# CarperAI/trlx

Measured on AMD Instinct MI355X. Metric: ppo_samples_per_sec, higher is better.
Workload: dtype bf16

## Files before the change

### trlx_amd/csrc/attn_host.h

```cpp
#pragma once

#include <ATen/ATen.h>

#include <string>
#include <type_traits>
#include <utility>

#include "dispatch.h"


template <int... Ds>
struct HeadDims {};
constexpr HeadDims<64, 96, 128, 256> kFlashHeadDims{};
constexpr HeadDims<64, 128> kSeq2SeqFlashHeadDims{};
constexpr HeadDims<32, 64, 96, 128, 256> kDecodeHeadDims{};
constexpr HeadDims<64, 128> kSeq2SeqDecodeHeadDims{};


template <int... Ds, typename F>
void dispatch_head_dim(HeadDims<Ds...>, int D, const char* op, F&& f) {
  const bool found = (... || (D == Ds ? (f(std::integral_constant<int, Ds>{}), true) : false));
  if (found) return;
  const int dims[] = {Ds...};
  const int n = sizeof...(Ds);
  std::string list;
  for (int i = 0; i < n; ++i)
    list += (i == 0 ? "" : i + 1 == n ? " or " : ", ") + std::to_string(dims[i]);
  TORCH_CHECK(false, op, ": head dim must be ", list, ", got ", D);
}

template <typename F>
void dispatch_flash_mode(int D, bool alibi, bool s2s_any, bool causal, bool rel_bias,
                         bool key_mask, const char* op, F&& f) {
  constexpr std::true_type yes{};
  constexpr std::false_type no{};
  if (s2s_any) {
    dispatch_head_dim(kSeq2SeqFlashHeadDims, D, op, [&](auto d) {
      dispatch_bool(causal, [&](auto ca) {
        dispatch_bool(rel_bias, [&](auto rb) {
          dispatch_bool(key_mask, [&](auto km) {
            constexpr bool plain =
                decltype(ca)::value && !decltype(rb)::value && !decltype(km)::value;
            if constexpr (!plain) f(d, no, ca, rb, km);
            else TORCH_INTERNAL_ASSERT(false, op, ": seq2seq dispatch without a seq2seq mode");
          });
        });
      });
    });
    return;
  }
  dispatch_head_dim(kFlashHeadDims, D, op, [&](auto d) {
    dispatch_bool(alibi, [&](auto al) { f(d, al, yes, no, no); });
  });
}


inline std::pair<at::Tensor, const int*> optional_int_ptr(const c10::optional<at::Tensor>& opt,
                                                          const at::Tensor& like, long B,
                                                          const char* op, const char* what) {
  if (!opt.has_value()) return {at::Tensor(), nullptr};
  TORCH_CHECK(opt->device() == like.device(), op, ": ", what,
              " must live on the same device as the inputs");
  TORCH_CHECK(opt->dtype() == at::kInt && opt->numel() == B, op, ": ", what,
              " must be int32 with one element per batch row (", B, "), got ", opt->dtype(),
              " x ", opt->numel());
  at::Tensor t = opt->contiguous();
  return {t, t.data_ptr<int>()};
}

inline const float* alibi_slopes_ptr(const c10::optional<at::Tensor>& slopes,
                                     const at::Tensor& like, long num_q_heads,
                                     const char* op) {
  if (!slopes.has_value()) return nullptr;
  TORCH_CHECK(slopes->dtype() == at::kFloat && slopes->is_contiguous(), op,
              ": alibi_slopes must be contiguous fp32");
  TORCH_CHECK(slopes->device() == like.device(), op,
              ": alibi_slopes must live on the same device as the inputs");
  TORCH_CHECK(slopes->numel() == num_q_heads, op, ": alibi_slopes needs one slope per query head (",
              num_q_heads, "), got ", slopes->numel());
  return slopes->data_ptr<float>();
}

struct Seq2SeqArgs {
  const float* rel_bias = nullptr;
  int bias_len = 0;
  int bias_zero = 0;
  const unsigned char* key_mask = nullptr;
  bool any = false;
};

inline Seq2SeqArgs seq2seq_args(const c10::optional<at::Tensor>& rel_bias, long bias_zero,
                                const c10::optional<at::Tensor>& key_mask, bool causal,
                                bool has_key_starts, bool has_alibi, const at::Tensor& like,
                                long B, long num_q_heads, long Tq, long Tk, long start_pos,
                                long D, const char* op) {
  Seq2SeqArgs a;
  if (rel_bias.has_value()) {
    TORCH_CHECK(!has_alibi, op, ": rel_bias and alibi_slopes are mutually exclusive");
    TORCH_CHECK(rel_bias->dtype() == at::kFloat && rel_bias->is_contiguous() &&
                    rel_bias->dim() == 2 && rel_bias->size(0) == num_q_heads,
                op, ": rel_bias must be contiguous fp32 [Hq, L]");
    TORCH_CHECK(rel_bias->device() == like.device(), op,
                ": rel_bias must live on the same device as the inputs");
    const long L = rel_bias->size(1);
    TORCH_CHECK(bias_zero - (start_pos + Tq - 1) >= 0 && bias_zero + Tk - 1 < L, op,
                ": rel_bias [Hq, ", L, "] with bias_zero ", bias_zero,
                " does not cover queries ", start_pos, "..", start_pos + Tq - 1, " x keys 0..",
                Tk - 1);
    a.rel_bias = rel_bias->data_ptr<float>();
    a.bias_len = (int)L;
    a.bias_zero = (int)bias_zero;
  }
  if (key_mask.has_value()) {
    TORCH_CHECK(!has_key_starts, op, ": key_mask and key_starts are mutually exclusive");
    TORCH_CHECK(key_mask->dtype() == at::kByte && key_mask->is_contiguous() &&
                    key_mask->dim() == 2 && key_mask->size(0) == B && key_mask->size(1) == Tk,
                op, ": key_mask must be contiguous uint8 [B, Tk]");
    TORCH_CHECK(key_mask->device() == like.device(), op,
                ": key_mask must live on the same device as the inputs");
    TORCH_CHECK(Tk > 0, op, ": key_mask needs at least one key");
    a.key_mask = key_mask->data_ptr<unsigned char>();
  }
  a.any = a.rel_bias != nullptr || a.key_mask != nullptr || !causal;
  if (a.any) {
    TORCH_CHECK(!has_alibi, op, ": key_mask / non-causal attention do not combine with alibi_slopes");
    TORCH_CHECK(D == 64 || D == 128, op,
                ": rel_bias / key_mask / non-causal attention need head dim 64 or 128, got ", D);
  }
  return a;
}
```

### trlx_amd/csrc/bindings.cpp

```cpp
#include <torch/extension.h>

std::vector<at::Tensor> logprobs_fwd(const at::Tensor& logits, const at::Tensor& labels);
at::Tensor logprobs_bwd(const at::Tensor& logits, const at::Tensor& labels, const at::Tensor& lse,
                        const at::Tensor& gout);
std::vector<at::Tensor> rmsnorm_fwd(const at::Tensor& x, const at::Tensor& w, double eps,
                                    const c10::optional<at::Tensor>& res);
std::vector<at::Tensor> rmsnorm_bwd(const at::Tensor& x, const at::Tensor& w,
                                    const at::Tensor& invr, const at::Tensor& dy,
                                    const c10::optional<at::Tensor>& dres);
std::vector<at::Tensor> layernorm_fwd(const at::Tensor& x, const at::Tensor& w,
                                      const c10::optional<at::Tensor>& b, double eps,
                                      const c10::optional<at::Tensor>& res);
std::vector<at::Tensor> layernorm_bwd(const at::Tensor& x, const at::Tensor& w,
                                      const at::Tensor& mean, const at::Tensor& invstd,
                                      const at::Tensor& dy,
                                      const c10::optional<at::Tensor>& dres);
at::Tensor rope_fwd(const at::Tensor& x, const at::Tensor& cos, const at::Tensor& sin,
                    const at::Tensor& pos, bool interleaved, bool inverse, long rot);
std::vector<at::Tensor> gae(const at::Tensor& values, const at::Tensor& rewards, double gamma,
                            double lam);
at::Tensor sum_count(const at::Tensor& x);
at::Tensor normalize(const at::Tensor& x, const at::Tensor& mean, const at::Tensor& var,
                     bool shift_mean);
std::vector<at::Tensor> ppo_loss(const at::Tensor& logprobs, const at::Tensor& values,
                                 const at::Tensor& old_logprobs, const at::Tensor& old_values,
                                 const at::Tensor& advantages, const at::Tensor& returns,
                                 const at::Tensor& mask, double cliprange, double cliprange_value,
                                 double vf_coef);
at::Tensor gumbel_sample(const at::Tensor& logits, double temperature,
                         const c10::optional<at::Tensor>& thresholds, long seed, long offset);
at::Tensor gumbel_sample_dev(const at::Tensor& logits, double temperature,
                             const c10::optional<at::Tensor>& thresholds, long seed,
                             const at::Tensor& offset);
at::Tensor decode_prep(const at::Tensor& qkv, at::Tensor& kcache, at::Tensor& vcache,
                       const c10::optional<at::Tensor>& cos, const c10::optional<at::Tensor>& sin,
                       const c10::optional<at::Tensor>& key_starts, const at::Tensor& cache_idx,
                       long num_heads, long rot, bool interleaved);
std::vector<at::Tensor> qkv_prep_fwd(const at::Tensor& qkv, long num_heads, long num_kv_heads,
                                     long head_dim, const c10::optional<at::Tensor>& cos,
                                     const c10::optional<at::Tensor>& sin,
                                     const c10::optional<at::Tensor>& pos, double qscale,
                                     long rot, bool interleaved);
at::Tensor qkv_prep_bwd(const at::Tensor& dq, const at::Tensor& dk, const at::Tensor& dv,
                        const c10::optional<at::Tensor>& cos, const c10::optional<at::Tensor>& sin,
                        const c10::optional<at::Tensor>& pos, double qscale, long rot,
                        bool interleaved);
at::Tensor causal_softmax_fwd(const at::Tensor& scores, long start_pos,
                              const c10::optional<at::Tensor>& key_starts);
at::Tensor causal_softmax_bwd(const at::Tensor& probs, const at::Tensor& dprobs);
at::Tensor attention_decode(const at::Tensor& q, const at::Tensor& kc, const at::Tensor& vc,
                            const at::Tensor& seq_lens, double scale,
                            const c10::optional<at::Tensor>& seq_starts,
                            const c10::optional<at::Tensor>& alibi_slopes);
at::Tensor lm_logprobs_v2(const at::Tensor& hidden, const at::Tensor& weight,
                          const at::Tensor& labels);
at::Tensor skinny_gemm(const at::Tensor& a, const at::Tensor& w,
                       const c10::optional<at::Tensor>& bias, long act);
at::Tensor skinny_gemm_fp8(const at::Tensor& a, const at::Tensor& w8, const at::Tensor& wscale,
                           const c10::optional<at::Tensor>& bias, long act);
std::vector<at::Tensor> lm_logprobs_v2_with_lse(const at::Tensor& hidden,
                                                const at::Tensor& weight,
                                                const at::Tensor& labels, bool want_lse);
at::Tensor ce_dlogits(const at::Tensor& hidden, const at::Tensor& weight,
                      const at::Tensor& labels, const at::Tensor& lse, const at::Tensor& dlp);
std::vector<at::Tensor> linear_gather_lse_fwd(const at::Tensor& x, const at::Tensor& w,
                                              const at::Tensor& bias, const at::Tensor& idx);
at::Tensor linear_gather_lse_bwd(const at::Tensor& x, const at::Tensor& w,
                                 const at::Tensor& bias, const at::Tensor& idx,
                                 const at::Tensor& lse, const at::Tensor& g_val,
                                 const at::Tensor& g_lse);
at::Tensor fused_decode_attention(const at::Tensor& qkv, at::Tensor& kcache, at::Tensor& vcache,
                                  const at::Tensor& seq_lens,
                                  const c10::optional<at::Tensor>& seq_starts,
                                  const c10::optional<at::Tensor>& cos,
                                  const c10::optional<at::Tensor>& sin,
                                  const at::Tensor& cache_idx, long rot, bool interleaved,
                                  double scale,
                                  const c10::optional<at::Tensor>& alibi_slopes);
void decode_advance(const at::Tensor& tok, at::Tensor& out_tokens, at::Tensor& cur_tok,
                    at::Tensor& finished, at::Tensor& rng_offset, at::Tensor& step_col,
                    at::Tensor& cache_idx, at::Tensor& seq_lens, at::Tensor& pos_ids,
                    const c10::optional<at::Tensor>& key_starts, long eos, long pad);
at::Tensor lm_logprobs(const at::Tensor& hidden, const at::Tensor& weight,
                       const at::Tensor& labels);
void fused_adamw(at::Tensor& p, at::Tensor& master, const at::Tensor& g, at::Tensor& m,
                 at::Tensor& v, long step, double lr, double beta1, double beta2, double eps,
                 double weight_decay, double grad_scale);
void stage_gemm(const at::Tensor& a, const at::Tensor& w, const c10::optional<at::Tensor>& bias,
                at::Tensor& c, const c10::optional<at::Tensor>& nstats,
                const c10::optional<at::Tensor>& nw, const c10::optional<at::Tensor>& nb,
                bool norm_rms, double eps, long act, const c10::optional<at::Tensor>& resid,
                const c10::optional<at::Tensor>& out_stats);
void embed_stats(const at::Tensor& wte, const c10::optional<at::Tensor>& wpe,
                 const at::Tensor& cur_tok, const at::Tensor& pos_ids, long pos_offset,
                 at::Tensor& x, at::Tensor& stats, at::Tensor& packed);
void lm_sample(const at::Tensor& x, const at::Tensor& wlm, const c10::optional<at::Tensor>& blm,
               const at::Tensor& nstats, const at::Tensor& nw,
               const c10::optional<at::Tensor>& nb, at::Tensor& packed, bool norm_rms,
               double eps, double temperature, long seed, const at::Tensor& rng_offset);
void advance_packed(const at::Tensor& packed, at::Tensor& out_tokens, at::Tensor& cur_tok,
                    at::Tensor& finished, at::Tensor& rng_offset, at::Tensor& step_col,
                    at::Tensor& cache_idx, at::Tensor& seq_lens, at::Tensor& pos_ids,
                    const c10::optional<at::Tensor>& key_starts, long eos, long pad);
void stage_gemm_v2(const at::Tensor& a, const at::Tensor& w, const c10::optional<at::Tensor>& bias,
                   at::Tensor& c, bool norm, const c10::optional<at::Tensor>& nw,
                   const c10::optional<at::Tensor>& nb, bool norm_rms, double eps, long act,
                   const c10::optional<at::Tensor>& resid,
                   const c10::optional<at::Tensor>& pstats_out);
void stage_gemm_v3(const at::Tensor& a, const at::Tensor& w, const c10::optional<at::Tensor>& bias,
                   at::Tensor& c, const c10::optional<at::Tensor>& pstats, long nparts,
                   const c10::optional<at::Tensor>& nw, const c10::optional<at::Tensor>& nb,
                   bool norm_rms, double eps, long act,
                   const c10::optional<at::Tensor>& pstats_out);
at::Tensor flash_prefill(const at::Tensor& q, const at::Tensor& k, const at::Tensor& v,
                         const c10::optional<at::Tensor>& key_starts, long start_pos,
                         double scale, long tk,
                         const c10::optional<at::Tensor>& alibi_slopes,
                         const c10::optional<at::Tensor>& rel_bias, long bias_zero,
                         const c10::optional<at::Tensor>& key_mask, bool causal);
std::vector<at::Tensor> flash_prefill_lse(const at::Tensor& q, const at::Tensor& k,
                                          const at::Tensor& v,
                                          const c10::optional<at::Tensor>& key_starts,
                                          long start_pos, double scale, long tk,
                                          bool want_lse,
                                          const c10::optional<at::Tensor>& alibi_slopes,
                                          const c10::optional<at::Tensor>& rel_bias, long bias_zero,
                                          const c10::optional<at::Tensor>& key_mask, bool causal);
std::vector<at::Tensor> flash_prefill_bwd(const at::Tensor& q, const at::Tensor& k,
                                          const at::Tensor& v, const at::Tensor& out,
                                          const at::Tensor& dout, const at::Tensor& lse,
                                          const c10::optional<at::Tensor>& key_starts,
                                          double scale,
                                          const c10::optional<at::Tensor>& alibi_slopes,
                                          const c10::optional<at::Tensor>& rel_bias, long bias_zero,
                                          const c10::optional<at::Tensor>& key_mask, bool causal);
at::Tensor seq2seq_decode_attention(const at::Tensor& q, const at::Tensor& k_new,
                                    const at::Tensor& v_new, at::Tensor& k_cache,
                                    at::Tensor& v_cache, const at::Tensor& cache_idx,
                                    const c10::optional<at::Tensor>& rel_bias, long bias_zero,
                                    double scale);
at::Tensor seq2seq_cross_decode_attention(const at::Tensor& q, const at::Tensor& k,
                                          const at::Tensor& v,
                                          const c10::optional<at::Tensor>& key_mask,
                                          double scale);
void lm_sample_v3(const at::Tensor& x, const at::Tensor& wlm,
                  const c10::optional<at::Tensor>& blm, const at::Tensor& pstats, long nparts,
                  const at::Tensor& nw, const c10::optional<at::Tensor>& nb, at::Tensor& packed,
                  bool norm_rms, double eps, double temperature, long seed,
                  const at::Tensor& rng_offset);
void lm_sample_v2(const at::Tensor& x, const at::Tensor& wlm,
                  const c10::optional<at::Tensor>& blm, const at::Tensor& nw,
                  const c10::optional<at::Tensor>& nb, at::Tensor& packed, bool norm_rms,
                  double eps, double temperature, long seed, const at::Tensor& rng_offset);

PYBIND11_MODULE(TORCH_EXTENSION_NAME, mod) {
  mod.def("logprobs_fwd", &logprobs_fwd, "fused logsumexp + label gather fwd");
  mod.def("logprobs_bwd", &logprobs_bwd, "logprobs backward");
  mod.def("rmsnorm_fwd", &rmsnorm_fwd);
  mod.def("rmsnorm_bwd", &rmsnorm_bwd);
  mod.def("layernorm_fwd", &layernorm_fwd);
  mod.def("layernorm_bwd", &layernorm_bwd);
  mod.def("rope_fwd", &rope_fwd);
  mod.def("gae", &gae);
  mod.def("sum_count", &sum_count);
  mod.def("normalize", &normalize);
  mod.def("ppo_loss", &ppo_loss);
  mod.def("gumbel_sample", &gumbel_sample);
  mod.def("gumbel_sample_dev", &gumbel_sample_dev);
  mod.def("decode_prep", &decode_prep);
  mod.def("qkv_prep_fwd", &qkv_prep_fwd);
  mod.def("qkv_prep_bwd", &qkv_prep_bwd);
  mod.def("causal_softmax_fwd", &causal_softmax_fwd);
  mod.def("causal_softmax_bwd", &causal_softmax_bwd);
  mod.def("attention_decode", &attention_decode, py::arg("q"), py::arg("k_cache"),
          py::arg("v_cache"), py::arg("seq_lens"), py::arg("scale"), py::arg("seq_starts"),
          py::arg("alibi_slopes") = py::none());
  mod.def("fused_adamw", &fused_adamw);
  mod.def("lm_logprobs", &lm_logprobs);
  mod.def("lm_logprobs_v2", &lm_logprobs_v2);
  mod.def("skinny_gemm", &skinny_gemm);
  mod.def("skinny_gemm_fp8", &skinny_gemm_fp8);
  mod.def("lm_logprobs_v2_with_lse", &lm_logprobs_v2_with_lse);
  mod.def("ce_dlogits", &ce_dlogits);
  mod.def("linear_gather_lse_fwd", &linear_gather_lse_fwd);
  mod.def("linear_gather_lse_bwd", &linear_gather_lse_bwd);
  mod.def("decode_advance", &decode_advance);
  mod.def("fused_decode_attention", &fused_decode_attention, py::arg("qkv"),
          py::arg("k_cache"), py::arg("v_cache"), py::arg("seq_lens"), py::arg("seq_starts"),
          py::arg("cos"), py::arg("sin"), py::arg("cache_idx"), py::arg("rot"),
          py::arg("interleaved"), py::arg("scale"), py::arg("alibi_slopes") = py::none());
  mod.def("stage_gemm", &stage_gemm);
  mod.def("embed_stats", &embed_stats);
  mod.def("lm_sample", &lm_sample);
  mod.def("advance_packed", &advance_packed);
  mod.def("stage_gemm_v2", &stage_gemm_v2);
  mod.def("lm_sample_v2", &lm_sample_v2);
  mod.def("stage_gemm_v3", &stage_gemm_v3);
  mod.def("lm_sample_v3", &lm_sample_v3);
  mod.def("flash_prefill", &flash_prefill, py::arg("q"), py::arg("k"), py::arg("v"),
          py::arg("key_starts"), py::arg("start_pos"), py::arg("scale"), py::arg("tk"),
          py::arg("alibi_slopes") = py::none(),
          py::arg("rel_bias") = py::none(), py::arg("bias_zero") = 0,
          py::arg("key_mask") = py::none(), py::arg("causal") = true);
  mod.def("flash_prefill_lse", &flash_prefill_lse, py::arg("q"), py::arg("k"), py::arg("v"),
          py::arg("key_starts"), py::arg("start_pos"), py::arg("scale"), py::arg("tk"),
          py::arg("want_lse"), py::arg("alibi_slopes") = py::none(),
          py::arg("rel_bias") = py::none(), py::arg("bias_zero") = 0,
          py::arg("key_mask") = py::none(), py::arg("causal") = true);
  mod.def("flash_prefill_bwd", &flash_prefill_bwd, py::arg("q"), py::arg("k"), py::arg("v"),
          py::arg("out"), py::arg("dout"), py::arg("lse"), py::arg("key_starts"),
          py::arg("scale"), py::arg("alibi_slopes") = py::none(),
          py::arg("rel_bias") = py::none(), py::arg("bias_zero") = 0,
          py::arg("key_mask") = py::none(), py::arg("causal") = true);
  mod.def("seq2seq_decode_attention", &seq2seq_decode_attention, py::arg("q"), py::arg("k_new"),
          py::arg("v_new"), py::arg("k_cache"), py::arg("v_cache"), py::arg("cache_idx"),
          py::arg("rel_bias") = py::none(), py::arg("bias_zero") = 0, py::arg("scale") = 1.0);
  mod.def("seq2seq_cross_decode_attention", &seq2seq_cross_decode_attention, py::arg("q"),
          py::arg("k"), py::arg("v"), py::arg("key_mask") = py::none(), py::arg("scale") = 1.0);
}
```

### trlx_amd/csrc/common.h

```cpp
#pragma once

#include <hip/hip_runtime.h>

#define WAVE 64
#define DEV __device__ __forceinline__

typedef __attribute__((ext_vector_type(2))) short short2v;
typedef __attribute__((ext_vector_type(4))) short short4v;
typedef __attribute__((ext_vector_type(8))) short short8v;
typedef __attribute__((ext_vector_type(4))) float float4v;


DEV float bf2f(unsigned short u) {
  union {
    float f;
    unsigned int i;
  } x;
  x.i = ((unsigned int)u) << 16;
  return x.f;
}

DEV unsigned short f2bf(float f) {
  union {
    float f;
    unsigned int i;
  } x;
  x.f = f;
  if ((x.i & 0x7fffffffu) > 0x7f800000u) return 0x7fc0;
  unsigned int lsb = (x.i >> 16) & 1u;
  x.i += 0x7fffu + lsb;
  return (unsigned short)(x.i >> 16);
}


template <typename T>
struct ScalarIO;

template <>
struct ScalarIO<float> {
  DEV static float load(const float* p) { return *p; }
  DEV static void store(float* p, float v) { *p = v; }
};

struct bf16_t {
  unsigned short u;
};

template <>
struct ScalarIO<bf16_t> {
  DEV static float load(const bf16_t* p) { return bf2f(p->u); }
  DEV static void store(bf16_t* p, float v) { p->u = f2bf(v); }
};

template <typename T>
DEV void load8(const T* p, float* out);

template <>
DEV void load8<float>(const float* p, float* out) {
  const float4v* v = reinterpret_cast<const float4v*>(p);
  float4v a = v[0], b = v[1];
#pragma unroll
  for (int i = 0; i < 4; ++i) {
    out[i] = a[i];
    out[i + 4] = b[i];
  }
}

template <>
DEV void load8<bf16_t>(const bf16_t* p, float* out) {
  short8v s = *reinterpret_cast<const short8v*>(p);
#pragma unroll
  for (int i = 0; i < 8; ++i) out[i] = bf2f((unsigned short)s[i]);
}

template <typename T>
DEV void store8(T* p, const float* in);

template <>
DEV void store8<float>(float* p, const float* in) {
  float4v a, b;
#pragma unroll
  for (int i = 0; i < 4; ++i) {
    a[i] = in[i];
    b[i] = in[i + 4];
  }
  float4v* v = reinterpret_cast<float4v*>(p);
  v[0] = a;
  v[1] = b;
}

template <>
DEV void store8<bf16_t>(bf16_t* p, const float* in) {
  short8v s;
#pragma unroll
  for (int i = 0; i < 8; ++i) s[i] = (short)f2bf(in[i]);
  *reinterpret_cast<short8v*>(p) = s;
}


DEV float wave_sum(float v) {
#pragma unroll
  for (int off = 32; off > 0; off >>= 1) v += __shfl_xor(v, off);
  return v;
}

DEV float wave_max(float v) {
#pragma unroll
  for (int off = 32; off > 0; off >>= 1) v = fmaxf(v, __shfl_xor(v, off));
  return v;
}

template <int NWAVES>
DEV float block_sum(float v, float* buf) {
  v = wave_sum(v);
  const int wid = threadIdx.x / WAVE;
  const int lane = threadIdx.x % WAVE;
  if (lane == 0) buf[wid] = v;
  __syncthreads();
  float r = 0.f;
#pragma unroll
  for (int i = 0; i < NWAVES; ++i) r += buf[i];
  __syncthreads();
  return r;
}

template <int NWAVES>
DEV float block_max(float v, float* buf) {
  v = wave_max(v);
  const int wid = threadIdx.x / WAVE;
  const int lane = threadIdx.x % WAVE;
  if (lane == 0) buf[wid] = v;
  __syncthreads();
  float r = -INFINITY;
#pragma unroll
  for (int i = 0; i < NWAVES; ++i) r = fmaxf(r, buf[i]);
  __syncthreads();
  return r;
}

struct MS {
  float m, s;
};

DEV MS ms_combine(MS a, MS b) {
  MS r;
  r.m = fmaxf(a.m, b.m);
  float ea = (a.m == -INFINITY) ? 0.f : __expf(a.m - r.m);
  float eb = (b.m == -INFINITY) ? 0.f : __expf(b.m - r.m);
  r.s = a.s * ea + b.s * eb;
  return r;
}

DEV MS wave_ms(MS v) {
#pragma unroll
  for (int off = 32; off > 0; off >>= 1) {
    MS o;
    o.m = __shfl_xor(v.m, off);
    o.s = __shfl_xor(v.s, off);
    v = ms_combine(v, o);
  }
  return v;
}


DEV float alibi_score(float score, float slope, int key, int kstart) {
  return __builtin_fmaf(slope, (float)(key - kstart), score);
}


DEV float rel_bias_score(float score, const float* __restrict__ bias_row, int L, int key,
                         int qpos, int bias_zero) {
  const int idx = min(max(key - qpos + bias_zero, 0), L - 1);
  return score + bias_row[idx];
}

struct S2SView {
  const float* rel_bias;
  int bias_len, bias_zero;
  const unsigned char* key_mask;
  int Tk;
};
constexpr bool s2s_pack_ok(bool any_flag, int pack_size, int expected) {
  return any_flag ? pack_size == expected : pack_size == 0;
}
DEV S2SView s2s_view() { return {nullptr, 0, 0, nullptr, 0}; }
DEV S2SView s2s_view(const float* rel_bias, int bias_len, int bias_zero,
                     const unsigned char* key_mask, int Tk = 0) {
  return {rel_bias, bias_len, bias_zero, key_mask, Tk};
}


DEV unsigned long long splitmix64(unsigned long long z) {
  z += 0x9e3779b97f4a7c15ull;
  z = (z ^ (z >> 30)) * 0xbf58476d1ce4e5b9ull;
  z = (z ^ (z >> 27)) * 0x94d049bb133111ebull;
  return z ^ (z >> 31);
}

DEV float rng_uniform(unsigned long long seed, unsigned long long a, unsigned long long b) {
  unsigned long long h = splitmix64(seed ^ splitmix64(a ^ splitmix64(b)));
  return ((h >> 40) + 1.0f) * (1.0f / 16777217.0f);
}

inline unsigned long long splitmix64_host(unsigned long long z) {
  z += 0x9e3779b97f4a7c15ull;
  z = (z ^ (z >> 30)) * 0xbf58476d1ce4e5b9ull;
  z = (z ^ (z >> 27)) * 0x94d049bb133111ebull;
  return z ^ (z >> 31);
}

#define HIP_CHECK_LAST()                                          \
  do {                                                             \
    hipError_t e = hipGetLastError();                              \
    TORCH_CHECK(e == hipSuccess, "HIP error: ", hipGetErrorString(e)); \
  } while (0)
```

### trlx_amd/csrc/flash_backward.hip

```cpp
#include <ATen/ATen.h>
#include <c10/hip/HIPStream.h>

#include "attn_host.h"
#include "common.h"

namespace {

constexpr int BBLOCK = 256;
constexpr int BT = 64;
constexpr int bwd_st(int D) { return D > 128 ? 32 : 64; }
constexpr int dkv_waves(int D) { return D > 128 ? 1 : 2; }

typedef __attribute__((ext_vector_type(8))) short bf16x8_fb;
typedef __attribute__((ext_vector_type(4))) float f32x4_fb;

template <int D, int ST>
DEV void stage_tileT(const bf16_t* __restrict__ src, long row0, long nrows,
                     unsigned short* __restrict__ tds, float mul) {
  constexpr int KPAD = ST + 8;
  for (int i = threadIdx.x; i < ST * (D / 8); i += BBLOCK) {
    const int row = i / (D / 8);
    const int col = (i % (D / 8)) * 8;
    const bf16_t* p = src + (size_t)(row0 + min((long)row, nrows - 1)) * D + col;
    bf16x8_fb v8 = *reinterpret_cast<const bf16x8_fb*>(p);
#pragma unroll
    for (int j = 0; j < 8; ++j) {
      float f = bf2f((unsigned short)v8[j]);
      tds[(col + j) * KPAD + row] = f2bf(mul == 1.f ? f : f * mul);
    }
  }
}

template <int D>
DEV void load_afrag(const bf16_t* __restrict__ src, long row0, long rowmax, int lane,
                    bf16x8_fb* frag, float mul) {
  const long row = min(row0 + (long)(lane & 15), rowmax);
  const int g8 = (lane >> 4) * 8;
#pragma unroll
  for (int dch = 0; dch < D / 32; ++dch) {
    bf16x8_fb v8 = *reinterpret_cast<const bf16x8_fb*>(src + (size_t)row * D + dch * 32 + g8);
    if (mul != 1.f) {
#pragma unroll
      for (int j = 0; j < 8; ++j) v8[j] = (short)f2bf(bf2f((unsigned short)v8[j]) * mul);
    }
    frag[dch] = v8;
  }
}

template <int KPAD>
DEV bf16x8_fb load_bfragT(const unsigned short* __restrict__ tds, int col, int dch, int g8) {
  bf16x8_fb r;
#pragma unroll
  for (int j = 0; j < 8; ++j) r[j] = (short)tds[(dch * 32 + g8 + j) * KPAD + col];
  return r;
}

template <int D, bool ALIBI, bool CAUSAL = true, bool RELB = false, bool KMASK = false,
          typename... S2S>
__global__ __launch_bounds__(BBLOCK, dkv_waves(D)) void flash_bwd_dkv_kernel(
    const bf16_t* __restrict__ q, const bf16_t* __restrict__ k, const bf16_t* __restrict__ v,
    const bf16_t* __restrict__ dout, const float* __restrict__ lse,
    const float* __restrict__ drow, const int* __restrict__ key_starts,
    const float* __restrict__ alibi_slopes ,
    bf16_t* __restrict__ dk, bf16_t* __restrict__ dv, int B, int Hq, int Hkv,
    int Tq , float scale,
    S2S... s2s_args ) {
  static_assert(s2s_pack_ok(!CAUSAL || RELB || KMASK, sizeof...(S2S), 5),
                "seq2seq arguments: (rel_bias, bias_len, bias_zero, key_mask, Tk) iff a mode is on");
  const S2SView s2s = s2s_view(s2s_args...);
  const float* __restrict__ rel_bias = s2s.rel_bias;
  const unsigned char* __restrict__ key_mask = s2s.key_mask;
  const int bias_len = s2s.bias_len, bias_zero = s2s.bias_zero;
  constexpr int ST = bwd_st(D);
  constexpr int KPAD = ST + 8;
  const int Tk = CAUSAL ? Tq : s2s.Tk;
  const int kt = blockIdx.x * BT;
  const int hkv = blockIdx.y;
  const int b = blockIdx.z;
  if (kt >= Tk) return;
  const int rep = Hq / Hkv;
  const int kstart = key_starts ? key_starts[b] : 0;

  const int lane = threadIdx.x % WAVE;
  const int wid = threadIdx.x / WAVE;
  const int c = lane & 15;
  const int g8 = (lane >> 4) * 8;
  const int krow0 = wid * 16;

  __shared__ unsigned short qT_lds[D * KPAD];
  __shared__ unsigned short doT_lds[D * KPAD];
  __shared__ float l_lds[ST];
  __shared__ float d_lds[ST];
  __shared__ unsigned short p_lds[BBLOCK / WAVE][16 * KPAD];

  bf16x8_fb k_frag[D / 32], v_frag[D / 32];
  load_afrag<D>(k + ((size_t)b * Hkv + hkv) * (size_t)Tk * D, kt + krow0, (long)Tk - 1, lane,
                k_frag, 1.f);
  load_afrag<D>(v + ((size_t)b * Hkv + hkv) * (size_t)Tk * D, kt + krow0, (long)Tk - 1, lane,
                v_frag, 1.f);
  bool kvis[4] = {true, true, true, true};
  if constexpr (KMASK) {
#pragma unroll
    for (int r = 0; r < 4; ++r)
      kvis[r] = key_mask[(size_t)b * Tk + min(kt + krow0 + (lane >> 4) * 4 + r, Tk - 1)] != 0;
  }

  f32x4_fb dv_acc[D / 16], dk_acc[D / 16];
#pragma unroll
  for (int d = 0; d < D / 16; ++d) {
    dv_acc[d] = {0.f, 0.f, 0.f, 0.f};
    dk_acc[d] = {0.f, 0.f, 0.f, 0.f};
  }

  for (int hq = hkv * rep; hq < (hkv + 1) * rep; ++hq) {
    const float slope = ALIBI ? alibi_slopes[hq] : 0.f;
    for (int qt = CAUSAL ? kt : 0; qt < Tq; qt += ST) {
      __syncthreads();
      stage_tileT<D, ST>(q + ((size_t)b * Hq + hq) * (size_t)Tq * D, qt, Tq - qt, qT_lds, scale);
      stage_tileT<D, ST>(dout + ((size_t)b * Hq + hq) * (size_t)Tq * D, qt, Tq - qt, doT_lds,
                         1.f);
      for (int i = threadIdx.x; i < ST; i += BBLOCK) {
        const int qrow = min(qt + i, Tq - 1);
        l_lds[i] = lse[((size_t)b * Hq + hq) * Tq + qrow];
        d_lds[i] = drow[((size_t)b * Hq + hq) * Tq + qrow];
      }
      __syncthreads();

      f32x4_fb pt[ST / 16], dst[ST / 16];
#pragma unroll
      for (int qq = 0; qq < ST / 16; ++qq) {
        f32x4_fb st = {0.f, 0.f, 0.f, 0.f};
        f32x4_fb dpt = {0.f, 0.f, 0.f, 0.f};
#pragma unroll
        for (int dch = 0; dch < D / 32; ++dch) {
          bf16x8_fb qf = load_bfragT<KPAD>(qT_lds, qq * 16 + c, dch, g8);
          st = __builtin_amdgcn_mfma_f32_16x16x32_bf16(k_frag[dch], qf, st, 0, 0, 0);
          bf16x8_fb df = load_bfragT<KPAD>(doT_lds, qq * 16 + c, dch, g8);
          dpt = __builtin_amdgcn_mfma_f32_16x16x32_bf16(v_frag[dch], df, dpt, 0, 0, 0);
        }
        const int qpos = qt + qq * 16 + c;
        const float L = l_lds[qq * 16 + c];
        const float Dr = d_lds[qq * 16 + c];
#pragma unroll
        for (int r = 0; r < 4; ++r) {
          const int key = kt + krow0 + (lane >> 4) * 4 + r;
          const bool valid = key < Tk && key >= kstart && (!CAUSAL || key <= qpos) &&
                             qpos < Tq && kvis[r];
          if constexpr (ALIBI) st[r] = alibi_score(st[r], slope, key, kstart);
          if constexpr (RELB)
            st[r] = rel_bias_score(st[r], rel_bias + (size_t)hq * bias_len, bias_len, key, qpos,
                                   bias_zero);
          const float p = (valid && L < INFINITY) ? __expf(st[r] - L) : 0.f;
          st[r] = p;
          dpt[r] = p * (dpt[r] - Dr);
        }
        pt[qq] = st;
        dst[qq] = dpt;
      }

      unsigned short* pw = p_lds[wid];
#pragma unroll
      for (int qq = 0; qq < ST / 16; ++qq)
#pragma unroll
        for (int r = 0; r < 4; ++r)
          pw[((lane >> 4) * 4 + r) * KPAD + qq * 16 + c] = f2bf(pt[qq][r]);
#pragma unroll
      for (int d = 0; d < D / 16; ++d)
#pragma unroll
        for (int qch = 0; qch < ST; qch += 32) {
          bf16x8_fb pf = *reinterpret_cast<const bf16x8_fb*>(&pw[c * KPAD + qch + g8]);
          bf16x8_fb dof =
              *reinterpret_cast<const bf16x8_fb*>(&doT_lds[(d * 16 + c) * KPAD + qch + g8]);
          dv_acc[d] = __builtin_amdgcn_mfma_f32_16x16x32_bf16(pf, dof, dv_acc[d], 0, 0, 0);
        }
#pragma unroll
      for (int qq = 0; qq < ST / 16; ++qq)
#pragma unroll
        for (int r = 0; r < 4; ++r)
          pw[((lane >> 4) * 4 + r) * KPAD + qq * 16 + c] = f2bf(dst[qq][r]);
#pragma unroll
      for (int d = 0; d < D / 16; ++d)
#pragma unroll
        for (int qch = 0; qch < ST; qch += 32) {
          bf16x8_fb sf = *reinterpret_cast<const bf16x8_fb*>(&pw[c * KPAD + qch + g8]);
          bf16x8_fb qtf =
              *reinterpret_cast<const bf16x8_fb*>(&qT_lds[(d * 16 + c) * KPAD + qch + g8]);
          dk_acc[d] = __builtin_amdgcn_mfma_f32_16x16x32_bf16(sf, qtf, dk_acc[d], 0, 0, 0);
        }
    }
  }

#pragma unroll
  for (int d = 0; d < D / 16; ++d)
#pragma unroll
    for (int r = 0; r < 4; ++r) {
      const int key = kt + krow0 + (lane >> 4) * 4 + r;
      if (key >= Tk) continue;
      dv[(((size_t)b * Hkv + hkv) * Tk + key) * D + d * 16 + c].u = f2bf(dv_acc[d][r]);
      dk[(((size_t)b * Hkv + hkv) * Tk + key) * D + d * 16 + c].u = f2bf(dk_acc[d][r]);
    }
}

template <int D, bool ALIBI, bool CAUSAL = true, bool RELB = false, bool KMASK = false,
          typename... S2S>
__global__ __launch_bounds__(BBLOCK, 2) void flash_bwd_dq_kernel(
    const bf16_t* __restrict__ q, const bf16_t* __restrict__ k, const bf16_t* __restrict__ v,
    const bf16_t* __restrict__ dout, const float* __restrict__ lse,
    const float* __restrict__ drow, const int* __restrict__ key_starts,
    const float* __restrict__ alibi_slopes ,
    bf16_t* __restrict__ dq, int B, int Hq, int Hkv,
    int Tq , float scale,
    S2S... s2s_args ) {
  static_assert(s2s_pack_ok(!CAUSAL || RELB || KMASK, sizeof...(S2S), 5),
                "seq2seq arguments: (rel_bias, bias_len, bias_zero, key_mask, Tk) iff a mode is on");
  const S2SView s2s = s2s_view(s2s_args...);
  const float* __restrict__ rel_bias = s2s.rel_bias;
  const unsigned char* __restrict__ key_mask = s2s.key_mask;
  const int bias_len = s2s.bias_len, bias_zero = s2s.bias_zero;
  constexpr int ST = bwd_st(D);
  constexpr int KPAD = ST + 8;
  const int Tk = CAUSAL ? Tq : s2s.Tk;
  const int qt = blockIdx.x * BT;
  const int h = blockIdx.y;
  const int b = blockIdx.z;
  if (qt >= Tq) return;
  const int hkv = h / (Hq / Hkv);
  const int kstart = key_starts ? key_starts[b] : 0;
  const float slope = ALIBI ? alibi_slopes[h] : 0.f;

  const int lane = threadIdx.x % WAVE;
  const int wid = threadIdx.x / WAVE;
  const int c = lane & 15;
  const int g8 = (lane >> 4) * 8;
  const int qrow0 = wid * 16;

  __shared__ unsigned short kT_lds[D * KPAD];
  __shared__ unsigned short vT_lds[D * KPAD];
  __shared__ unsigned short p_lds[BBLOCK / WAVE][16 * KPAD];

  bf16x8_fb q_frag[D / 32], do_frag[D / 32];
  load_afrag<D>(q + ((size_t)b * Hq + h) * (size_t)Tq * D, qt + qrow0, (long)Tq - 1, lane,
                q_frag, scale);
  load_afrag<D>(dout + ((size_t)b * Hq + h) * (size_t)Tq * D, qt + qrow0, (long)Tq - 1, lane,
                do_frag, 1.f);
  float L_r[4], D_r[4];
#pragma unroll
  for (int r = 0; r < 4; ++r) {
    const int qrow = min(qt + qrow0 + (lane >> 4) * 4 + r, Tq - 1);
    L_r[r] = lse[((size_t)b * Hq + h) * Tq + qrow];
    D_r[r] = drow[((size_t)b * Hq + h) * Tq + qrow];
  }

  f32x4_fb dq_acc[D / 16];
#pragma unroll
  for (int d = 0; d < D / 16; ++d) dq_acc[d] = {0.f, 0.f, 0.f, 0.f};

  const int kt_lo = (kstart / ST) * ST;
  const int kt_hi = CAUSAL ? min(Tk, qt + BT) : Tk;
  for (int kt = kt_lo; kt < kt_hi; kt += ST) {
    __syncthreads();
    stage_tileT<D, ST>(k + ((size_t)b * Hkv + hkv) * (size_t)Tk * D, kt, Tk - kt, kT_lds, 1.f);
    stage_tileT<D, ST>(v + ((size_t)b * Hkv + hkv) * (size_t)Tk * D, kt, Tk - kt, vT_lds, 1.f);
    __syncthreads();

    unsigned short* pw = p_lds[wid];
#pragma unroll
    for (int kk = 0; kk < ST / 16; ++kk) {
      f32x4_fb s = {0.f, 0.f, 0.f, 0.f};
      f32x4_fb dp = {0.f, 0.f, 0.f, 0.f};
#pragma unroll
      for (int dch = 0; dch < D / 32; ++dch) {
        bf16x8_fb kf = load_bfragT<KPAD>(kT_lds, kk * 16 + c, dch, g8);
        s = __builtin_amdgcn_mfma_f32_16x16x32_bf16(q_frag[dch], kf, s, 0, 0, 0);
        bf16x8_fb vf = load_bfragT<KPAD>(vT_lds, kk * 16 + c, dch, g8);
        dp = __builtin_amdgcn_mfma_f32_16x16x32_bf16(do_frag[dch], vf, dp, 0, 0, 0);
      }
      const int key = kt + kk * 16 + c;
      bool kvis = true;
      if constexpr (KMASK) kvis = key_mask[(size_t)b * Tk + min(key, Tk - 1)] != 0;
#pragma unroll
      for (int r = 0; r < 4; ++r) {
        const int qrow = qt + qrow0 + (lane >> 4) * 4 + r;
        const bool valid = key < Tk && key >= kstart && (!CAUSAL || key <= qrow) &&
                           qrow < Tq && kvis;
        if constexpr (ALIBI) s[r] = alibi_score(s[r], slope, key, kstart);
        if constexpr (RELB)
          s[r] = rel_bias_score(s[r], rel_bias + (size_t)h * bias_len, bias_len, key, qrow,
                                bias_zero);
        const float p = (valid && L_r[r] < INFINITY) ? __expf(s[r] - L_r[r]) : 0.f;
        s[r] = p * (dp[r] - D_r[r]);
      }
#pragma unroll
      for (int r = 0; r < 4; ++r)
        pw[((lane >> 4) * 4 + r) * KPAD + kk * 16 + c] = f2bf(s[r]);
    }
#pragma unroll
    for (int d = 0; d < D / 16; ++d)
#pragma unroll
      for (int kch = 0; kch < ST; kch += 32) {
        bf16x8_fb sf = *reinterpret_cast<const bf16x8_fb*>(&pw[c * KPAD + kch + g8]);
        bf16x8_fb ktf =
            *reinterpret_cast<const bf16x8_fb*>(&kT_lds[(d * 16 + c) * KPAD + kch + g8]);
        dq_acc[d] = __builtin_amdgcn_mfma_f32_16x16x32_bf16(sf, ktf, dq_acc[d], 0, 0, 0);
      }
  }

#pragma unroll
  for (int d = 0; d < D / 16; ++d)
#pragma unroll
    for (int r = 0; r < 4; ++r) {
      const int qrow = qt + qrow0 + (lane >> 4) * 4 + r;
      if (qrow >= Tq) continue;
      dq[(((size_t)b * Hq + h) * Tq + qrow) * D + d * 16 + c].u = f2bf(scale * dq_acc[d][r]);
    }
}

}

std::vector<at::Tensor> flash_prefill_bwd(const at::Tensor& q, const at::Tensor& k,
                                          const at::Tensor& v, const at::Tensor& out,
                                          const at::Tensor& dout, const at::Tensor& lse,
                                          const c10::optional<at::Tensor>& key_starts,
                                          double scale,
                                          const c10::optional<at::Tensor>& alibi_slopes,
                                          const c10::optional<at::Tensor>& rel_bias,
                                          long bias_zero,
                                          const c10::optional<at::Tensor>& key_mask,
                                          bool causal) {
  TORCH_CHECK(q.is_cuda() && q.dtype() == at::kBFloat16 && q.dim() == 4 && q.is_contiguous(),
              "flash_prefill_bwd: q must be contiguous bf16 [B,Hq,T,D]");
  TORCH_CHECK(k.is_contiguous() && v.is_contiguous() && lse.is_contiguous());
  const int B = q.size(0), Hq = q.size(1), T = q.size(2), D = q.size(3);
  const int Hkv = k.size(1), Tk = k.size(2);
  TORCH_CHECK(!causal || Tk == T, "flash_prefill_bwd: training path only (Tk == T)");
  TORCH_CHECK(Hq % Hkv == 0 && k.size(3) == D && v.sizes() == k.sizes());
  TORCH_CHECK(out.sizes() == q.sizes() && dout.sizes() == q.sizes() && lse.numel() == (long)B * Hq * T);
  const float* sl = alibi_slopes_ptr(alibi_slopes, q, Hq, "flash_prefill_bwd");
  const Seq2SeqArgs s2s =
      seq2seq_args(rel_bias, bias_zero, key_mask, causal, key_starts.has_value(), sl != nullptr,
                   q, B, Hq, T, Tk, 0, D, "flash_prefill_bwd");
  const auto ks_t = optional_int_ptr(key_starts, q, B, "flash_prefill_bwd", "key_starts");
  const int* ks = ks_t.second;
  auto dq = at::empty_like(q);
  auto dk = at::empty_like(k);
  auto dv = at::empty_like(v);
  auto dc = dout.contiguous();
  auto drow = (dc.to(at::kFloat) * out.to(at::kFloat)).sum(-1).contiguous();
  auto stream = c10::hip::getCurrentHIPStream();
  auto qp = reinterpret_cast<const bf16_t*>(q.data_ptr());
  auto kp = reinterpret_cast<const bf16_t*>(k.data_ptr());
  auto vp = reinterpret_cast<const bf16_t*>(v.data_ptr());
  auto dop = reinterpret_cast<const bf16_t*>(dc.data_ptr());
  auto dqp = reinterpret_cast<bf16_t*>(dq.data_ptr());
  auto dkp = reinterpret_cast<bf16_t*>(dk.data_ptr());
  auto dvp = reinterpret_cast<bf16_t*>(dv.data_ptr());
  const float* lp = lse.data_ptr<float>();
  const float* drp = drow.data_ptr<float>();
  dim3 gk((Tk + BT - 1) / BT, Hkv, B);
  dim3 gq((T + BT - 1) / BT, Hq, B);
  dispatch_flash_mode(
      D, sl != nullptr, s2s.any, causal, s2s.rel_bias != nullptr, s2s.key_mask != nullptr,
      "flash_prefill_bwd", [&](auto d, auto al, auto ca, auto rb, auto km) {
        constexpr int DV = decltype(d)::value;
        constexpr bool AL = decltype(al)::value, CA = decltype(ca)::value,
                       RB = decltype(rb)::value, KM = decltype(km)::value;
        auto launch = [&](auto... s2s_pack) {
          flash_bwd_dkv_kernel<DV, AL, CA, RB, KM><<<gk, BBLOCK, 0, stream>>>(
              qp, kp, vp, dop, lp, drp, ks, sl, dkp, dvp, B, Hq, Hkv, T, (float)scale,
              s2s_pack...);
          flash_bwd_dq_kernel<DV, AL, CA, RB, KM><<<gq, BBLOCK, 0, stream>>>(
              qp, kp, vp, dop, lp, drp, ks, sl, dqp, B, Hq, Hkv, T, (float)scale, s2s_pack...);
        };
        if constexpr (CA && !RB && !KM) launch();
        else launch(s2s.rel_bias, s2s.bias_len, s2s.bias_zero, s2s.key_mask, Tk);
      });
  HIP_CHECK_LAST();
  return {dq, dk, dv};
}
```

### trlx_amd/csrc/flash_prefill.hip

```cpp
#include <ATen/ATen.h>
#include <c10/hip/HIPStream.h>

#include "attn_host.h"
#include "common.h"

namespace {

constexpr int FBLOCK = 256;
constexpr int FWAVES = FBLOCK / WAVE;
constexpr int TQ = 64;
constexpr int fwd_tk(int D) { return D > 128 ? 32 : 64; }

typedef __attribute__((ext_vector_type(8))) short bf16x8_fp;
typedef __attribute__((ext_vector_type(4))) float f32x4_fp;

template <int D, bool ALIBI, bool CAUSAL = true, bool RELB = false, bool KMASK = false,
          typename... S2S>
__global__ __launch_bounds__(FBLOCK, 2) void flash_prefill_kernel(
    const bf16_t* __restrict__ q, const bf16_t* __restrict__ k, const bf16_t* __restrict__ v,
    const int* __restrict__ key_starts,
    const float* __restrict__ alibi_slopes ,
    bf16_t* __restrict__ out,
    float* __restrict__ lse ,
    int B, int Hq, int Hkv, int T, int Tk,
    int Sk , int start_pos, float scale,
    S2S... s2s_args) {
  static_assert(s2s_pack_ok(!CAUSAL || RELB || KMASK, sizeof...(S2S), 4),
                "seq2seq arguments: (rel_bias, bias_len, bias_zero, key_mask) iff a mode is on");
  const S2SView s2s = s2s_view(s2s_args...);
  const float* __restrict__ rel_bias = s2s.rel_bias;
  const unsigned char* __restrict__ key_mask = s2s.key_mask;
  const int bias_len = s2s.bias_len, bias_zero = s2s.bias_zero;
  constexpr int TK = fwd_tk(D);
  constexpr bool QREG = D > 128;
  constexpr int DPAD = D + 8;
  constexpr int KPAD = TK + 8;

  const int qt = blockIdx.x;
  const int h = blockIdx.y;
  const int b = blockIdx.z;
  const int hkv = h / (Hq / Hkv);
  const int q0 = qt * TQ;
  if (q0 >= T) return;
  const int kstart = key_starts ? key_starts[b] : 0;
  const float slope = ALIBI ? alibi_slopes[h] : 0.f;

  const int lane = threadIdx.x % WAVE;
  const int wid = threadIdx.x / WAVE;

  __shared__ unsigned short q_lds[QREG ? 8 : TQ * DPAD];
  __shared__ unsigned short k_lds[TK * DPAD];
  __shared__ unsigned short vt_lds[D * KPAD];
  __shared__ unsigned short p_lds[FWAVES][16 * KPAD];

  bf16x8_fp q_frag[QREG ? D / 32 : 1];
  if constexpr (QREG) {
    const int qrow = min(q0 + wid * 16 + (lane & 15), T - 1);
    const bf16_t* qp = q + (((size_t)b * Hq + h) * T + qrow) * D + (lane >> 4) * 8;
#pragma unroll
    for (int dch = 0; dch < D / 32; ++dch) {
      float vals[8];
      load8<bf16_t>(qp + dch * 32, vals);
#pragma unroll
      for (int j = 0; j < 8; ++j) q_frag[dch][j] = (short)f2bf(vals[j] * scale);
    }
  } else {
    const bf16_t* qp = q + (((size_t)b * Hq + h) * T) * D;
    for (int i = threadIdx.x; i < TQ * (D / 8); i += FBLOCK) {
      const int row = i / (D / 8);
      const int col = (i % (D / 8)) * 8;
      const int qrow = min(q0 + row, T - 1);
      float vals[8];
      load8<bf16_t>(qp + (size_t)qrow * D + col, vals);
      bf16x8_fp s;
#pragma unroll
      for (int j = 0; j < 8; ++j) s[j] = (short)f2bf(vals[j] * scale);
      *reinterpret_cast<bf16x8_fp*>(&q_lds[row * DPAD + col]) = s;
    }
  }
  __syncthreads();

  const int qrow0 = wid * 16;
  const int qhi_pos = start_pos + min(q0 + TQ - 1, T - 1);

  float m_row[4], l_row[4];
#pragma unroll
  for (int r = 0; r < 4; ++r) {
    m_row[r] = -INFINITY;
    l_row[r] = 0.f;
  }
  f32x4_fp oacc[D / 16];
#pragma unroll
  for (int d = 0; d < D / 16; ++d) oacc[d] = {0.f, 0.f, 0.f, 0.f};

  const bf16_t* kp = k + (((size_t)b * Hkv + hkv) * (size_t)Sk) * D;
  const bf16_t* vp = v + (((size_t)b * Hkv + hkv) * (size_t)Sk) * D;

  const int kt_lo = (kstart / TK) * TK;
  const int kt_hi = CAUSAL ? min(Tk, qhi_pos + 1) : Tk;

  for (int kt = kt_lo; kt < kt_hi; kt += TK) {
    __syncthreads();
    for (int i = threadIdx.x; i < TK * (D / 8); i += FBLOCK) {
      const int row = i / (D / 8);
      const int col = (i % (D / 8)) * 8;
      const int krow = min(kt + row, Tk - 1);
      bf16x8_fp kv8 = *reinterpret_cast<const bf16x8_fp*>(kp + (size_t)krow * D + col);
      *reinterpret_cast<bf16x8_fp*>(&k_lds[row * DPAD + col]) = kv8;
      bf16x8_fp vv8 = *reinterpret_cast<const bf16x8_fp*>(vp + (size_t)krow * D + col);
#pragma unroll
      for (int j = 0; j < 8; ++j) vt_lds[(col + j) * KPAD + row] = (unsigned short)vv8[j];
    }
    __syncthreads();

    const int c = lane & 15;
    const int g8 = (lane >> 4) * 8;
    f32x4_fp sfrag[TK / 16];
#pragma unroll
    for (int kk = 0; kk < TK / 16; ++kk) {
      f32x4_fp acc = {0.f, 0.f, 0.f, 0.f};
#pragma unroll
      for (int d = 0; d < D; d += 32) {
        bf16x8_fp af;
        if constexpr (QREG) af = q_frag[d / 32];
        else af = *reinterpret_cast<const bf16x8_fp*>(&q_lds[(qrow0 + c) * DPAD + d + g8]);
        bf16x8_fp bf = *reinterpret_cast<const bf16x8_fp*>(&k_lds[(kk * 16 + c) * DPAD + d + g8]);
        acc = __builtin_amdgcn_mfma_f32_16x16x32_bf16(af, bf, acc, 0, 0, 0);
      }
      sfrag[kk] = acc;
    }

    float mnew[4];
#pragma unroll
    for (int r = 0; r < 4; ++r) mnew[r] = m_row[r];
#pragma unroll
    for (int kk = 0; kk < TK / 16; ++kk) {
      const int key = kt + kk * 16 + c;
      if constexpr (ALIBI) {
#pragma unroll
        for (int r = 0; r < 4; ++r) sfrag[kk][r] = alibi_score(sfrag[kk][r], slope, key, kstart);
      }
      if constexpr (RELB) {
#pragma unroll
        for (int r = 0; r < 4; ++r)
          sfrag[kk][r] = rel_bias_score(sfrag[kk][r], rel_bias + (size_t)h * bias_len, bias_len,
                                        key, start_pos + q0 + qrow0 + (lane >> 4) * 4 + r,
                                        bias_zero);
      }
      bool kvis = true;
      if constexpr (KMASK) kvis = key_mask[(size_t)b * Tk + min(key, Tk - 1)] != 0;
#pragma unroll
      for (int r = 0; r < 4; ++r) {
        const int qrow = q0 + qrow0 + (lane >> 4) * 4 + r;
        const bool valid = key < Tk && key >= kstart && (!CAUSAL || key <= start_pos + qrow) &&
                           qrow < T && kvis;
        if (!valid) sfrag[kk][r] = -INFINITY;
      }
    }
#pragma unroll
    for (int r = 0; r < 4; ++r) {
      float mx = -INFINITY;
#pragma unroll
      for (int kk = 0; kk < TK / 16; ++kk) mx = fmaxf(mx, sfrag[kk][r]);
#pragma unroll
      for (int off = 8; off > 0; off >>= 1) mx = fmaxf(mx, __shfl_xor(mx, off));
      mnew[r] = fmaxf(mnew[r], mx);
    }
    float psum[4] = {0.f, 0.f, 0.f, 0.f};
#pragma unroll
    for (int kk = 0; kk < TK / 16; ++kk) {
#pragma unroll
      for (int r = 0; r < 4; ++r) {
        const float p = (sfrag[kk][r] == -INFINITY || mnew[r] == -INFINITY)
                            ? 0.f
                            : __expf(sfrag[kk][r] - mnew[r]);
        sfrag[kk][r] = p;
        psum[r] += p;
        p_lds[wid][((lane >> 4) * 4 + r) * KPAD + kk * 16 + c] = f2bf(p);
      }
    }
#pragma unroll
    for (int r = 0; r < 4; ++r) {
#pragma unroll
      for (int off = 8; off > 0; off >>= 1) psum[r] += __shfl_xor(psum[r], off);
    }

    float corr[4];
#pragma unroll
    for (int r = 0; r < 4; ++r) {
      corr[r] = (m_row[r] == -INFINITY || mnew[r] == -INFINITY) ? 0.f
                : __expf(m_row[r] - mnew[r]);
      l_row[r] = l_row[r] * corr[r] + psum[r];
      m_row[r] = mnew[r];
    }
#pragma unroll
    for (int d = 0; d < D / 16; ++d) {
#pragma unroll
      for (int r = 0; r < 4; ++r) oacc[d][r] *= corr[r];
    }
#pragma unroll
    for (int d = 0; d < D / 16; ++d) {
#pragma unroll
      for (int kk2 = 0; kk2 < TK; kk2 += 32) {
        bf16x8_fp pf = *reinterpret_cast<const bf16x8_fp*>(&p_lds[wid][c * KPAD + kk2 + g8]);
        bf16x8_fp vf = *reinterpret_cast<const bf16x8_fp*>(&vt_lds[(d * 16 + c) * KPAD + kk2 + g8]);
        oacc[d] = __builtin_amdgcn_mfma_f32_16x16x32_bf16(pf, vf, oacc[d], 0, 0, 0);
      }
    }
  }

  const int c = lane & 15;
  if (lse != nullptr && c == 0) {
#pragma unroll
    for (int r = 0; r < 4; ++r) {
      const int qrow = q0 + qrow0 + (lane >> 4) * 4 + r;
      if (qrow < T) {
        const float L = l_row[r] > 0.f ? m_row[r] + __logf(l_row[r]) : INFINITY;
        lse[((size_t)b * Hq + h) * T + qrow] = L;
      }
    }
  }
#pragma unroll
  for (int d = 0; d < D / 16; ++d) {
#pragma unroll
    for (int r = 0; r < 4; ++r) {
      const int qrow = q0 + qrow0 + (lane >> 4) * 4 + r;
      if (qrow >= T) continue;
      const float denom = l_row[r] > 0.f ? l_row[r] : 1.f;
      const float val = oacc[d][r] / denom;
      out[(((size_t)b * Hq + h) * T + qrow) * D + d * 16 + c].u = f2bf(val);
    }
  }
}

}

std::vector<at::Tensor> flash_prefill_lse(const at::Tensor& q, const at::Tensor& k,
                                          const at::Tensor& v,
                                          const c10::optional<at::Tensor>& key_starts,
                                          long start_pos, double scale, long tk, bool want_lse,
                                          const c10::optional<at::Tensor>& alibi_slopes,
                                          const c10::optional<at::Tensor>& rel_bias,
                                          long bias_zero,
                                          const c10::optional<at::Tensor>& key_mask, bool causal);

at::Tensor flash_prefill(const at::Tensor& q, const at::Tensor& k, const at::Tensor& v,
                         const c10::optional<at::Tensor>& key_starts, long start_pos,
                         double scale, long tk,
                         const c10::optional<at::Tensor>& alibi_slopes,
                         const c10::optional<at::Tensor>& rel_bias, long bias_zero,
                         const c10::optional<at::Tensor>& key_mask, bool causal) {
  return flash_prefill_lse(q, k, v, key_starts, start_pos, scale, tk, false, alibi_slopes,
                           rel_bias, bias_zero, key_mask, causal)[0];
}

std::vector<at::Tensor> flash_prefill_lse(const at::Tensor& q, const at::Tensor& k,
                                          const at::Tensor& v,
                                          const c10::optional<at::Tensor>& key_starts,
                                          long start_pos, double scale, long tk,
                                          bool want_lse,
                                          const c10::optional<at::Tensor>& alibi_slopes,
                                          const c10::optional<at::Tensor>& rel_bias,
                                          long bias_zero,
                                          const c10::optional<at::Tensor>& key_mask,
                                          bool causal) {
  TORCH_CHECK(q.is_cuda() && q.dtype() == at::kBFloat16 && q.dim() == 4 && q.is_contiguous());
  TORCH_CHECK(k.is_contiguous() && v.is_contiguous());
  const int B = q.size(0), Hq = q.size(1), T = q.size(2), D = q.size(3);
  const int Hkv = k.size(1), Sk = k.size(2);
  const int Tk = tk > 0 ? (int)tk : Sk;
  TORCH_CHECK(Tk <= Sk);
  TORCH_CHECK(k.size(3) == D && Hq % Hkv == 0);
  const float* sl = alibi_slopes_ptr(alibi_slopes, q, Hq, "flash_prefill");
  const Seq2SeqArgs s2s =
      seq2seq_args(rel_bias, bias_zero, key_mask, causal, key_starts.has_value(), sl != nullptr,
                   q, B, Hq, T, Tk, start_pos, D, "flash_prefill");
  auto out = at::empty_like(q);
  auto lse = want_lse ? at::empty({B, Hq, T}, q.options().dtype(at::kFloat)) : at::Tensor();
  if (q.numel() == 0) return {out, lse};
  const auto ks_t = optional_int_ptr(key_starts, q, B, "flash_prefill", "key_starts");
  const int* ks = ks_t.second;
  auto stream = c10::hip::getCurrentHIPStream();
  dim3 grid((T + TQ - 1) / TQ, Hq, B);
  auto qp = reinterpret_cast<const bf16_t*>(q.data_ptr());
  auto kp = reinterpret_cast<const bf16_t*>(k.data_ptr());
  auto vp = reinterpret_cast<const bf16_t*>(v.data_ptr());
  auto op = reinterpret_cast<bf16_t*>(out.data_ptr());
  float* lp = want_lse ? lse.data_ptr<float>() : nullptr;
  dispatch_flash_mode(
      D, sl != nullptr, s2s.any, causal, s2s.rel_bias != nullptr, s2s.key_mask != nullptr,
      "flash_prefill", [&](auto d, auto al, auto ca, auto rb, auto km) {
        constexpr int DV = decltype(d)::value;
        constexpr bool AL = decltype(al)::value, CA = decltype(ca)::value,
                       RB = decltype(rb)::value, KM = decltype(km)::value;
        auto launch = [&](auto... s2s_pack) {
          flash_prefill_kernel<DV, AL, CA, RB, KM><<<grid, FBLOCK, 0, stream>>>(
              qp, kp, vp, ks, sl, op, lp, B, Hq, Hkv, T, Tk, Sk, (int)start_pos, (float)scale,
              s2s_pack...);
        };
        if constexpr (CA && !RB && !KM) launch();
        else launch(s2s.rel_bias, s2s.bias_len, s2s.bias_zero, s2s.key_mask);
      });
  HIP_CHECK_LAST();
  return {out, lse};
}
```

### trlx_amd/models/nn/transformer.py

```python

import math
from dataclasses import dataclass
from typing import List, Optional, Tuple

import torch
import torch.nn as nn
import torch.nn.functional as F

from ... import ops
from ...ops.reference import rope_cos_sin
from ...parallel import topo
from ...parallel.tp import ColumnParallelLinear, RowParallelLinear
from .config import TransformerConfig


class Norm(nn.Module):

    def __init__(self, cfg: TransformerConfig, hidden: Optional[int] = None):
        super().__init__()
        h = hidden or cfg.hidden_size
        self.kind = cfg.norm
        self.eps = cfg.norm_eps
        self.weight = nn.Parameter(torch.ones(h))
        self.bias = nn.Parameter(torch.zeros(h)) if cfg.norm == "layernorm" else None

    def forward(self, x):
        if self.kind == "rmsnorm":
            return ops.rmsnorm(x, self.weight, self.eps)
        return ops.layernorm(x, self.weight, self.bias, self.eps)

    def forward_add(self, x, res):
        if self.kind == "rmsnorm":
            return ops.rmsnorm_add(x, res, self.weight, self.eps)
        return ops.layernorm_add(x, res, self.weight, self.bias, self.eps)


def alibi_slopes(num_heads: int) -> torch.Tensor:

    def pow2_slopes(n):
        start = 2.0 ** (-(2.0 ** -(math.log2(n) - 3)))
        return [start * (start ** i) for i in range(n)]

    if math.log2(num_heads).is_integer():
        vals = pow2_slopes(num_heads)
    else:
        closest = 2 ** math.floor(math.log2(num_heads))
        vals = pow2_slopes(closest) + pow2_slopes(2 * closest)[0::2][: num_heads - closest]
    return torch.tensor(vals, dtype=torch.float32)


@dataclass
class AttentionContext:

    position_ids: torch.Tensor
    key_starts: Optional[torch.Tensor]
    start_pos: int
    seq_lens: Optional[torch.Tensor] = None
    cache_idx: Optional[torch.Tensor] = None
    cache_rows: Optional[torch.Tensor] = None
    alibi_slopes: Optional[torch.Tensor] = None
    alibi: Optional[torch.Tensor] = None
    prefix_kv: Optional[object] = None
    virtual_slots: Optional[torch.Tensor] = None

    def dense_alibi(self, batch: int, num_keys: int) -> torch.Tensor:
        if self.alibi is None or self.alibi.shape[-1] != num_keys:
            slopes = self.alibi_slopes
            j = torch.arange(num_keys, device=slopes.device).unsqueeze(0)
            ks = (self.key_starts.unsqueeze(1) if self.key_starts is not None
                  else torch.zeros(batch, 1, device=slopes.device))
            key_pos = (j - ks).clamp(min=0).float()
            self.alibi = slopes.view(1, -1, 1, 1) * key_pos[:, None, None, :]
        return self.alibi


class KVCache:

    def __init__(self, num_layers: int, batch: int, num_kv_heads: int, max_len: int, head_dim: int,
                 device, dtype):
        self.k = [
            torch.zeros(batch, num_kv_heads, max_len, head_dim, device=device, dtype=dtype)
            for _ in range(num_layers)
        ]
        self.v = [
            torch.zeros(batch, num_kv_heads, max_len, head_dim, device=device, dtype=dtype)
            for _ in range(num_layers)
        ]
        self.max_len = max_len
        self.cur_len = 0

    def update(self, layer: int, k: torch.Tensor, v: torch.Tensor, start: int) -> Tuple[torch.Tensor, torch.Tensor]:
        T = k.shape[2]
        assert start + T <= self.max_len, "KV cache overflow"
        self.k[layer][:, :, start : start + T] = k
        self.v[layer][:, :, start : start + T] = v
        return self.k[layer], self.v[layer]

    def update_rows(self, layer: int, k: torch.Tensor, v: torch.Tensor,
                    rows: torch.Tensor) -> Tuple[torch.Tensor, torch.Tensor]:
        b = torch.arange(k.shape[0], device=k.device)
        self.k[layer][b, :, rows.long()] = k[:, :, 0]
        self.v[layer][b, :, rows.long()] = v[:, :, 0]
        return self.k[layer], self.v[layer]


class Attention(nn.Module):
    def __init__(self, cfg: TransformerConfig, layer_idx: int):
        super().__init__()
        self.cfg = cfg
        self.layer_idx = layer_idx
        tp = topo.tp_size()
        assert cfg.num_heads % tp == 0 and cfg.num_kv_heads % tp == 0, \
            f"heads ({cfg.num_heads}/{cfg.num_kv_heads}) must divide tp={tp}"
        self.num_heads = cfg.num_heads // tp
        self.num_kv_heads = cfg.num_kv_heads // tp
        self.head_dim = cfg.head_dim
        self.scale = cfg.attn_scale if cfg.attn_scale is not None else 1.0 / math.sqrt(cfg.head_dim)
        if tp > 1:
            self.qkv_proj = ColumnParallelLinear(cfg.hidden_size, cfg.qkv_out, bias=cfg.attn_bias)
            self.o_proj = RowParallelLinear(cfg.num_heads * cfg.head_dim, cfg.hidden_size,
                                            bias=cfg.attn_bias)
        else:
            self.qkv_proj = nn.Linear(cfg.hidden_size, cfg.qkv_out, bias=cfg.attn_bias)
            self.o_proj = nn.Linear(cfg.num_heads * cfg.head_dim, cfg.hidden_size, bias=cfg.attn_bias)
        self.rot = int(cfg.head_dim * cfg.rope_pct) if cfg.position_encoding == "rope" else 0
        if self.rot % 2:
            self.rot -= 1
        self.attn_pdrop = cfg.attn_pdrop

    def forward(self, x, ctx: AttentionContext, rope_tables, kv_cache: Optional[KVCache] = None):
        B = x.shape[0]
        qkv = dense(self.qkv_proj, x)
        T = qkv.shape[1]

        def project(out):
            return dense(self.o_proj, out.transpose(1, 2).reshape(B, T, -1))

        if (T == 1 and kv_cache is not None and ctx.cache_idx is not None
                and ctx.seq_lens is not None and x.is_cuda
                and self.head_dim in ops.DECODE_HEAD_DIMS):
            cos_sin = rope_tables if self.cfg.position_encoding == "rope" else (None, None)
            if self.num_heads == self.num_kv_heads:
                out = ops.fused_decode_attention(
                    qkv, kv_cache.k[self.layer_idx], kv_cache.v[self.layer_idx],
                    ctx.seq_lens, ctx.key_starts, cos_sin[0], cos_sin[1], ctx.cache_idx,
                    self.rot, self.cfg.rope_interleaved, self.scale,
                    alibi_slopes=ctx.alibi_slopes,
                )
            else:
                q = ops.decode_prep(
                    qkv, kv_cache.k[self.layer_idx], kv_cache.v[self.layer_idx], ctx.cache_idx,
                    self.num_heads, cos_sin[0], cos_sin[1], ctx.key_starts, self.rot,
                    self.cfg.rope_interleaved,
                )
                out = ops.attention_decode(q, kv_cache.k[self.layer_idx],
                                           kv_cache.v[self.layer_idx],
                                           ctx.seq_lens, self.scale, seq_starts=ctx.key_starts,
                                           alibi_slopes=ctx.alibi_slopes)
            return project(out)

        if x.is_cuda and x.dtype == torch.bfloat16 and ops.extension_available():
            use_rope = self.cfg.position_encoding == "rope"
            cos, sin = rope_tables if use_rope else (None, None)
            q, k, v = ops.qkv_prep(
                qkv, self.num_heads, self.num_kv_heads, self.head_dim, cos, sin,
                positions=ctx.position_ids if use_rope else None, qscale=self.scale,
                rot=self.rot, interleaved=self.cfg.rope_interleaved,
            )
            pre_scaled = True
        else:
            qd = self.num_heads * self.head_dim
            kd = self.num_kv_heads * self.head_dim
            q = qkv[..., :qd].view(B, T, self.num_heads, self.head_dim).transpose(1, 2).contiguous()
            k = qkv[..., qd : qd + kd].view(B, T, self.num_kv_heads, self.head_dim).transpose(1, 2).contiguous()
            v = qkv[..., qd + kd :].view(B, T, self.num_kv_heads, self.head_dim).transpose(1, 2).contiguous()
            pre_scaled = False

            if self.cfg.position_encoding == "rope":
                cos, sin = rope_tables
                q, k = ops.apply_rope(q, k, cos, sin, positions=ctx.position_ids,
                                      interleaved=self.cfg.rope_interleaved, rot=self.rot)

        if ctx.prefix_kv is not None:
            pk = ctx.prefix_kv.prefix_k[self.layer_idx].to(k.dtype)
            pv = ctx.prefix_kv.prefix_v[self.layer_idx].to(v.dtype)
            B_, n_ = ctx.virtual_slots.shape
            idx = ctx.virtual_slots.view(B_, 1, n_, 1).expand(B_, k.shape[1], n_, k.shape[3])
            k = k.scatter(2, idx, pk.unsqueeze(0).expand(B_, -1, -1, -1))
            v = v.scatter(2, idx, pv.unsqueeze(0).expand(B_, -1, -1, -1))

        flash_common = (
            T > 1 and x.is_cuda and q.dtype == torch.bfloat16
            and (self.attn_pdrop == 0 or not self.training)
            and ops.extension_available()
        )
        flash_ok = (
            flash_common and not torch.is_grad_enabled()
            and ops.flash_enabled(self.head_dim, train=False)
        )
        if kv_cache is not None:
            if pre_scaled:
                pass
            if ctx.cache_rows is not None:
                k_full, v_full = kv_cache.update_rows(self.layer_idx, k, v, ctx.cache_rows)
            else:
                k_full, v_full = kv_cache.update(self.layer_idx, k, v, ctx.start_pos)
            if (T == 1 and ctx.seq_lens is not None
                    and (not x.is_cuda or self.head_dim in ops.DECODE_HEAD_DIMS)):
                out = ops.attention_decode(q, k_full, v_full, ctx.seq_lens,
                                           1.0 if pre_scaled else self.scale,
                                           seq_starts=ctx.key_starts,
                                           alibi_slopes=ctx.alibi_slopes)
                return project(out)
            if flash_ok:
                out = ops.flash_prefill(q, k_full, v_full, ctx.key_starts, ctx.start_pos,
                                        1.0 if pre_scaled else self.scale,
                                        tk=ctx.start_pos + T, alibi_slopes=ctx.alibi_slopes)
                return project(out)
            k = k_full[:, :, : ctx.start_pos + T]
            v = v_full[:, :, : ctx.start_pos + T]
        elif flash_ok:
            out = ops.flash_prefill(q.contiguous(), k.contiguous(), v.contiguous(),
                                    ctx.key_starts, ctx.start_pos,
                                    1.0 if pre_scaled else self.scale,
                                    alibi_slopes=ctx.alibi_slopes)
            return project(out)

        flash_train_ok = (
            flash_common and torch.is_grad_enabled() and kv_cache is None and ctx.start_pos == 0
            and ops.flash_enabled(self.head_dim, train=True)
        )
        if flash_train_ok:
            out = ops.flash_attention(q, k, v, ctx.key_starts,
                                      1.0 if pre_scaled else self.scale,
                                      alibi_slopes=ctx.alibi_slopes)
            return project(out)

        if self.num_kv_heads != self.num_heads:
            rep = self.num_heads // self.num_kv_heads
            k = k.repeat_interleave(rep, dim=1)
            v = v.repeat_interleave(rep, dim=1)
        qs = q if pre_scaled else q * self.scale
        scores = torch.matmul(qs, k.transpose(-1, -2))
        if ctx.alibi_slopes is not None:
            scores = scores + ctx.dense_alibi(B, scores.shape[-1]).to(scores.dtype)
        probs = ops.causal_softmax(scores.contiguous(), ctx.start_pos, ctx.key_starts)
        if self.attn_pdrop > 0 and self.training:
            probs = F.dropout(probs, self.attn_pdrop)
        out = torch.matmul(probs, v)
        return project(out)


def dense(lin, x, act_code=0, act_fn=None):
    if type(lin) is nn.Linear:
        return ops.skinny_linear(x, lin.weight, lin.bias, act_code)
    y = lin(x)
    return act_fn(y) if act_fn is not None else y


_ACTS = {
    "gelu": F.gelu,
    "gelu_new": lambda x: F.gelu(x, approximate="tanh"),
    "relu": F.relu,
    "silu": F.silu,
}


class MLP(nn.Module):
    def __init__(self, cfg: TransformerConfig):
        super().__init__()
        self.swiglu = cfg.swiglu
        tp = topo.tp_size()
        i = cfg.intermediate_size
        assert i % tp == 0, f"intermediate {i} must divide tp={tp}"
        if tp > 1:
            if cfg.swiglu:
                self.gate_up_proj = ColumnParallelLinear(cfg.hidden_size, 2 * i, bias=cfg.mlp_bias)
            else:
                self.fc_in = ColumnParallelLinear(cfg.hidden_size, i, bias=cfg.mlp_bias)
            self.down_proj = RowParallelLinear(i, cfg.hidden_size, bias=cfg.mlp_bias)
        else:
            if cfg.swiglu:
                self.gate_up_proj = nn.Linear(cfg.hidden_size, 2 * i, bias=cfg.mlp_bias)
            else:
                self.fc_in = nn.Linear(cfg.hidden_size, i, bias=cfg.mlp_bias)
            self.down_proj = nn.Linear(i, cfg.hidden_size, bias=cfg.mlp_bias)
        self.act = _ACTS[cfg.activation]
        self.act_code = ops.ACT_CODES.get(cfg.activation)
        self.isize = i // tp

    def forward(self, x):
        if self.swiglu:
            gu = dense(self.gate_up_proj, x)
            return dense(self.down_proj, self.act(gu[..., : self.isize]) * gu[..., self.isize :])
        if self.act_code is None:
            return dense(self.down_proj, self.act(dense(self.fc_in, x)))
        return dense(self.down_proj, dense(self.fc_in, x, self.act_code, self.act))


class Block(nn.Module):
    def __init__(self, cfg: TransformerConfig, layer_idx: int):
        super().__init__()
        self.cfg = cfg
        self.ln_1 = Norm(cfg)
        self.attn = Attention(cfg, layer_idx)
        self.shared_parallel_norm = cfg.parallel_residual and cfg.arch_name == "gptj"
        if not self.shared_parallel_norm:
            self.ln_2 = Norm(cfg)
        self.mlp = MLP(cfg)
        self.resid_pdrop = cfg.resid_pdrop

    def _drop(self, x):
        if self.resid_pdrop > 0 and self.training:
            return F.dropout(x, self.resid_pdrop)
        return x

    def forward(self, x, ctx, rope_tables, kv_cache=None, res=None):
        if self.cfg.parallel_residual:
            if res is None:
                s = x
                h1 = self.ln_1(x)
            else:
                h1, s = self.ln_1.forward_add(x, res)
            h2 = h1 if self.shared_parallel_norm else self.ln_2(s)
            out = self._drop(self.attn(h1, ctx, rope_tables, kv_cache)) + self._drop(self.mlp(h2))
            return out, s
        if res is None:
            s = x
            h1 = self.ln_1(x)
        else:
            h1, s = self.ln_1.forward_add(x, res)
        a = self._drop(self.attn(h1, ctx, rope_tables, kv_cache))
        h2, s2 = self.ln_2.forward_add(a, s)
        m = self._drop(self.mlp(h2))
        return m, s2


def insert_virtual_rows(h, attention_mask, n, virt_values=None):
    B, T, H = h.shape
    device = h.device
    if attention_mask is not None:
        p = (T - attention_mask.sum(-1)).long()
    else:
        p = torch.zeros(B, dtype=torch.long, device=device)
    pos = torch.arange(T + n, device=device).unsqueeze(0)
    pe = p.unsqueeze(1)
    is_virt = (pos >= pe) & (pos < pe + n)
    src = torch.where(pos < pe, pos, (pos - n).clamp(min=0)).clamp(max=T - 1)
    h2 = torch.gather(h, 1, src.unsqueeze(-1).expand(B, T + n, H))
    if virt_values is not None:
        virt_idx = (pos - pe).clamp(0, n - 1)
        vfill = virt_values[virt_idx]
        h2 = torch.where(is_virt.unsqueeze(-1), vfill.to(h2.dtype), h2)
    else:
        h2 = h2.masked_fill(is_virt.unsqueeze(-1), 0)
    if attention_mask is not None:
        mask2 = torch.where(is_virt, torch.ones_like(is_virt, dtype=attention_mask.dtype),
                            torch.gather(attention_mask, 1, src))
    else:
        mask2 = is_virt.to(torch.long) | (pos >= pe + n).to(torch.long)
        mask2 = torch.ones(B, T + n, dtype=torch.long, device=device)
    slots = pe + torch.arange(n, device=device).unsqueeze(0)
    t_pos = torch.arange(T, device=device).unsqueeze(0)
    strip_idx = torch.where(t_pos < pe, t_pos, t_pos + n)
    return h2, mask2, slots, strip_idx


def _strip_virtual(t, strip_idx):
    if t is None:
        return None
    B, T = strip_idx.shape
    if t.dim() == 3:
        return torch.gather(t, 1, strip_idx.unsqueeze(-1).expand(B, T, t.shape[-1]))
    return torch.gather(t, 1, strip_idx)


@dataclass
class TransformerOutput:
    logits: Optional[torch.Tensor] = None
    last_hidden_state: Optional[torch.Tensor] = None
    hidden_at_layer: Optional[torch.Tensor] = None


class CausalTransformer(nn.Module):

    def __init__(self, config: TransformerConfig):
        super().__init__()
        self.config = config
        cfg = config
        self.embed_tokens = nn.Embedding(cfg.vocab_size, cfg.hidden_size)
        if cfg.position_encoding == "learned":
            off = cfg.extra.get("position_offset", 0)
            self.embed_positions = nn.Embedding(cfg.max_position_embeddings + off, cfg.hidden_size)
        else:
            self.embed_positions = None
        self.embed_norm = Norm(cfg) if cfg.extra.get("pre_embed_norm") else None
        self.layers = nn.ModuleList(Block(cfg, i) for i in range(cfg.num_layers))
        self.final_norm = Norm(cfg)
        self.lm_head = nn.Linear(cfg.hidden_size, cfg.vocab_size, bias=cfg.lm_head_bias)
        if cfg.tie_word_embeddings:
            self.lm_head.weight = self.embed_tokens.weight
        self.embd_pdrop = cfg.embd_pdrop
        self.gradient_checkpointing = False
        self.soft_prompt = None
        self.prefix_kv = None
        self.num_virtual_tokens = 0
        if cfg.position_encoding == "rope":
            rot = int(cfg.head_dim * cfg.rope_pct)
            rot -= rot % 2
            cos, sin = rope_cos_sin(cfg.max_position_embeddings, rot, cfg.rope_base)
            self.register_buffer("rope_cos", cos, persistent=False)
            self.register_buffer("rope_sin", sin, persistent=False)
        else:
            self.rope_cos = self.rope_sin = None
        self.register_buffer("alibi_slopes", self._local_alibi_slopes(), persistent=False)
        self.sequence_parallel = False
        self.apply(self._init_weights)

    def _local_alibi_slopes(self) -> Optional[torch.Tensor]:
        if self.config.position_encoding != "alibi":
            return None
        slopes = alibi_slopes(self.config.num_heads)
        tp = topo.tp_size()
        if tp > 1:
            hl = self.config.num_heads // tp
            slopes = slopes[topo.tp_rank() * hl : (topo.tp_rank() + 1) * hl].contiguous()
        return slopes

    def _apply(self, fn, *args, **kwargs):
        super()._apply(fn, *args, **kwargs)
        buf = self._buffers.get("alibi_slopes")
        if buf is not None and buf.dtype != torch.float32:
            self._buffers["alibi_slopes"] = self._local_alibi_slopes().to(buf.device)
        return self

    def set_sequence_parallel(self, enabled: bool):
        from ...parallel.tp import ColumnParallelLinear, RowParallelLinear

        self.sequence_parallel = enabled
        for m in self.modules():
            if isinstance(m, (ColumnParallelLinear, RowParallelLinear)):
                m.sequence_parallel = enabled

    def _init_weights(self, module):
        if isinstance(module, (nn.Linear, ColumnParallelLinear, RowParallelLinear)):
            module.weight.data.normal_(mean=0.0, std=0.02)
            if module.bias is not None:
                module.bias.data.zero_()
        elif isinstance(module, nn.Embedding):
            module.weight.data.normal_(mean=0.0, std=0.02)


    def _sp_flags_on(self) -> bool:
        from ...parallel.tp import ColumnParallelLinear

        for m in self.modules():
            if isinstance(m, ColumnParallelLinear):
                return m.sequence_parallel
        return False

    def _set_sp_flags(self, enabled: bool):
        from ...parallel.tp import ColumnParallelLinear, RowParallelLinear

        for m in self.modules():
            if isinstance(m, (ColumnParallelLinear, RowParallelLinear)):
                m.sequence_parallel = enabled

    def embed_parameters(self):
        params = list(self.embed_tokens.parameters())
        if self.embed_positions is not None:
            params += list(self.embed_positions.parameters())
        return params

    @property
    def rope_tables(self):
        return (self.rope_cos, self.rope_sin) if self.rope_cos is not None else None

    def make_context(self, input_ids, attention_mask, start_pos: int,
                     seq_lens: Optional[torch.Tensor] = None,
                     key_starts: Optional[torch.Tensor] = None,
                     position_ids: Optional[torch.Tensor] = None) -> AttentionContext:
        B, T = input_ids.shape[:2]
        device = input_ids.device
        if position_ids is not None:
            position_ids = position_ids.to(torch.int32)
        elif attention_mask is not None:
            mask = attention_mask.to(torch.int32)
            position_ids = (mask.cumsum(-1) - 1).clamp(min=0).to(torch.int32)
            key_starts = (T - mask.sum(-1)).to(torch.int32)
        else:
            position_ids = (
                torch.arange(start_pos, start_pos + T, device=device, dtype=torch.int32)
                .unsqueeze(0).expand(B, T).contiguous()
            )
        return AttentionContext(position_ids=position_ids, key_starts=key_starts,
                                start_pos=start_pos, seq_lens=seq_lens,
                                alibi_slopes=self.alibi_slopes)

    def run_layers(self, h, ctx, kv_cache=None, from_layer: int = 0, to_layer: Optional[int] = None):
        to_layer = len(self.layers) if to_layer is None else to_layer
        res = None
        for i in range(from_layer, to_layer):
            h, res = self.layers[i](h, ctx, self.rope_tables, kv_cache, res=res)
        return h if res is None else h + res


    def forward(
        self,
        input_ids: torch.Tensor,
        attention_mask: Optional[torch.Tensor] = None,
        position_ids: Optional[torch.Tensor] = None,
        kv_cache: Optional[KVCache] = None,
        start_pos: int = 0,
        seq_lens: Optional[torch.Tensor] = None,
        key_starts: Optional[torch.Tensor] = None,
        hidden_at_layer: Optional[int] = None,
        return_logits: bool = True,
        cache_idx: Optional[torch.Tensor] = None,
        cache_rows: Optional[torch.Tensor] = None,
        logits_slice: Optional[Tuple[int, int]] = None,
    ) -> TransformerOutput:
        nv = self.num_virtual_tokens if (self.soft_prompt is not None
                                         or self.prefix_kv is not None) else 0
        strip_idx = None
        if nv and start_pos == 0 and cache_idx is None:
            h = self.embed_tokens(input_ids)
            virt = self.soft_prompt.embeddings if self.soft_prompt is not None else None
            h, attention_mask, slots, strip_idx = insert_virtual_rows(h, attention_mask, nv, virt)
            ctx = self.make_context(h[..., 0], attention_mask, start_pos, seq_lens, None, None)
            ctx.cache_idx = cache_idx
            if self.prefix_kv is not None:
                ctx.prefix_kv = self.prefix_kv
                ctx.virtual_slots = slots
        else:
            ctx = self.make_context(input_ids, attention_mask, start_pos, seq_lens, key_starts,
                                    position_ids)
            ctx.cache_idx = cache_idx
            ctx.cache_rows = cache_rows
            h = self.embed_tokens(input_ids)
        if self.embed_norm is not None:
            h = self.embed_norm(h)
        if self.embed_positions is not None:
            off = self.config.extra.get("position_offset", 0)
            h = h + self.embed_positions(ctx.position_ids.long() + off)
        if self.embd_pdrop > 0 and self.training:
            h = F.dropout(h, self.embd_pdrop)

        sp_active = (self.sequence_parallel and topo.tp_size() > 1 and kv_cache is None
                     and input_ids.shape[1] % topo.tp_size() == 0)
        if sp_active != self._sp_flags_on():
            self._set_sp_flags(sp_active)
        if sp_active:
            from ...parallel.tp import scatter_to_sp

            h = scatter_to_sp(h)

        n = len(self.layers)
        multi = isinstance(hidden_at_layer, (list, tuple))
        wanted = list(hidden_at_layer) if multi else (
            [hidden_at_layer] if hidden_at_layer is not None else [])
        stash_for = {}
        for w in wanted:
            stash_for.setdefault(w % n, []).append(w)
        hidden_at = {} if multi else None
        res = None
        use_ckpt = self.gradient_checkpointing and self.training and torch.is_grad_enabled()
        for i, layer in enumerate(self.layers):
            if i in stash_for:
                stream = h if res is None else h + res
                if multi:
                    for w in stash_for[i]:
                        hidden_at[w] = stream
                else:
                    hidden_at = stream
            if use_ckpt:
                h, res = torch.utils.checkpoint.checkpoint(
                    lambda hh, rr, _l=layer: _l(hh, ctx, self.rope_tables, kv_cache, res=rr),
                    h, res, use_reentrant=False)
            else:
                h, res = layer(h, ctx, self.rope_tables, kv_cache, res=res)
        if res is None:
            h = self.final_norm(h)
        else:
            h, _ = self.final_norm.forward_add(h, res)
        if sp_active:
            from ...parallel.tp import gather_from_sp_replicated

            h = gather_from_sp_replicated(h)
            if isinstance(hidden_at, dict):
                hidden_at = {k: gather_from_sp_replicated(v) for k, v in hidden_at.items()}
            elif hidden_at is not None:
                hidden_at = gather_from_sp_replicated(hidden_at)
        if strip_idx is not None:
            h = _strip_virtual(h, strip_idx)
            if isinstance(hidden_at, dict):
                hidden_at = {kk: _strip_virtual(v, strip_idx) for kk, v in hidden_at.items()}
            elif hidden_at is not None:
                hidden_at = _strip_virtual(hidden_at, strip_idx)
        logits = None
        if return_logits:
            hs = h if logits_slice is None else h[:, logits_slice[0] : logits_slice[1]].contiguous()
            logits = self.lm_head(hs)
        return TransformerOutput(logits=logits, last_hidden_state=h, hidden_at_layer=hidden_at)

    def new_kv_cache(self, batch: int, max_len: int, device=None, dtype=None) -> KVCache:
        p = next(self.parameters())
        kv_heads_local = self.config.num_kv_heads // topo.tp_size()
        return KVCache(len(self.layers), batch, kv_heads_local, max_len,
                       self.config.head_dim, device or p.device, dtype or p.dtype)

    def num_parameters(self) -> int:
        return sum(p.numel() for p in self.parameters())
```

### trlx_amd/ops/__init__.py

```python

import os
from typing import Optional, Tuple

import torch

from . import reference

FLASH_HEAD_DIMS = (64, 96, 128, 256)
DECODE_HEAD_DIMS = (32, 64, 96, 128, 256)

FLASH_PREFILL_DEFAULT_DIMS = (64, 96, 128)
FLASH_TRAIN_DEFAULT_DIMS = (64, 128)

SEQ2SEQ_FLASH_HEAD_DIMS = (64, 128)
SEQ2SEQ_FLASH_PREFILL_DEFAULT_DIMS = (64, 128)
SEQ2SEQ_FLASH_TRAIN_DEFAULT_DIMS = (64, 128)

SEQ2SEQ_DECODE_HEAD_DIMS = (64, 128)


def _flash_gate(head_dim: int, train: bool, built, prefill_default, train_default) -> bool:
    if head_dim not in built:
        return False
    prefill = os.environ.get("TRLX_AMD_NO_FLASH_PREFILL")
    if prefill == "1":
        return False
    if not train:
        return prefill == "0" or head_dim in prefill_default
    switch = os.environ.get("TRLX_AMD_NO_FLASH_TRAIN")
    if switch == "1":
        return False
    return switch == "0" or head_dim in train_default


def flash_enabled(head_dim: int, train: bool) -> bool:
    return _flash_gate(head_dim, train, FLASH_HEAD_DIMS, FLASH_PREFILL_DEFAULT_DIMS,
                       FLASH_TRAIN_DEFAULT_DIMS)


def seq2seq_flash_enabled(head_dim: int, train: bool) -> bool:
    return _flash_gate(head_dim, train, SEQ2SEQ_FLASH_HEAD_DIMS,
                       SEQ2SEQ_FLASH_PREFILL_DEFAULT_DIMS, SEQ2SEQ_FLASH_TRAIN_DEFAULT_DIMS)


_EXT = None
_EXT_TRIED = False
_EXT_ERR: Optional[str] = None


def _load_ext():
    global _EXT, _EXT_TRIED, _EXT_ERR
    if _EXT_TRIED:
        return _EXT
    _EXT_TRIED = True
    try:
        from trlx_amd import _C

        _EXT = _C
    except ImportError as e:
        _EXT = None
        _EXT_ERR = str(e)
    return _EXT


def extension_available() -> bool:
    return _load_ext() is not None


def _require_ext(op_name: str):
    ext = _load_ext()
    if ext is None:
        if os.environ.get("TRLX_AMD_ALLOW_EAGER") == "1":
            return None
        raise RuntimeError(
            f"trlx_amd op '{op_name}' needs the HIP extension (trlx_amd._C) on GPU "
            f"but it is not built (import error: {_EXT_ERR}). "
            f"Run `python setup.py build_ext --inplace` (or __graft_entry__.build()). "
            f"Set TRLX_AMD_ALLOW_EAGER=1 to debug with the eager fallback."
        )
    return ext




class _LogprobsOfLabels(torch.autograd.Function):
    @staticmethod
    def forward(ctx, logits, labels, ext):
        logprobs, lse = ext.logprobs_fwd(logits, labels)
        ctx.save_for_backward(logits, labels, lse)
        return logprobs

    @staticmethod
    def backward(ctx, grad_out):
        logits, labels, lse = ctx.saved_tensors
        ext = _require_ext("logprobs_of_labels")
        grad_logits = ext.logprobs_bwd(logits, labels, lse, grad_out.contiguous())
        return grad_logits, None, None


def logprobs_of_labels(logits: torch.Tensor, labels: torch.Tensor) -> torch.Tensor:
    if logits.is_cuda:
        ext = _require_ext("logprobs_of_labels")
        if ext is not None:
            flat_logits = logits.reshape(-1, logits.shape[-1]).contiguous()
            flat_labels = labels.reshape(-1).contiguous()
            out = _LogprobsOfLabels.apply(flat_logits, flat_labels, ext)
            return out.view(labels.shape)
    return reference.logprobs_of_labels(logits, labels)




def lm_logprobs(hidden: torch.Tensor, weight: torch.Tensor, labels: torch.Tensor) -> torch.Tensor:
    if hidden.is_cuda:
        ext = _require_ext("lm_logprobs")
        if ext is not None and hasattr(ext, "lm_logprobs"):
            h = hidden.contiguous()
            if h.shape[1] % 64 == 0 and hasattr(ext, "lm_logprobs_v2") and \
                    os.environ.get("TRLX_AMD_LM_LOGPROBS_V1") != "1":
                return ext.lm_logprobs_v2(h, weight.contiguous(), labels.contiguous())
            return ext.lm_logprobs(h, weight.contiguous(), labels.contiguous())
    logits = hidden.float() @ weight.float().t()
    return reference.logprobs_of_labels(logits, labels)


class _LMLogprobsTrain(torch.autograd.Function):

    @staticmethod
    def forward(ctx, hidden, weight, labels, ext):
        out, lse = ext.lm_logprobs_v2_with_lse(hidden, weight, labels, True)
        ctx.save_for_backward(hidden, weight, labels, lse)
        return out

    @staticmethod
    def backward(ctx, grad_out):
        hidden, weight, labels, lse = ctx.saved_tensors
        ext = _require_ext("lm_logprobs_train")
        dlogits = ext.ce_dlogits(hidden, weight, labels, lse,
                                 grad_out.contiguous().float())
        dh = dlogits @ weight
        dw = dlogits.t() @ hidden if ctx.needs_input_grad[1] else None
        return dh, dw, None, None


def lm_logprobs_train(hidden: torch.Tensor, weight: torch.Tensor,
                      labels: torch.Tensor) -> torch.Tensor:
    if (hidden.is_cuda and hidden.dtype == torch.bfloat16
            and weight.dtype == torch.bfloat16 and hidden.shape[-1] % 64 == 0
            and os.environ.get("TRLX_AMD_FUSED_LM_LOGPROBS") != "0"):
        ext = _require_ext("lm_logprobs_train")
        if ext is not None and hasattr(ext, "ce_dlogits"):
            return _LMLogprobsTrain.apply(hidden.contiguous(), weight.contiguous(),
                                          labels.contiguous(), ext)
    logits = torch.nn.functional.linear(hidden, weight)
    return logprobs_of_labels(logits, labels)


class _LinearGatherLSE(torch.autograd.Function):

    @staticmethod
    def forward(ctx, x, weight, bias, idx, ext):
        xb = x.to(torch.bfloat16).contiguous()
        wb = weight.to(torch.bfloat16).contiguous()
        b = bias.float().contiguous()
        val, lse = ext.linear_gather_lse_fwd(xb, wb, b, idx)
        ctx.save_for_backward(xb, wb, b, idx, lse)
        ctx.in_dtypes = (x.dtype, weight.dtype, bias.dtype)
        return val, lse

    @staticmethod
    def backward(ctx, g_val, g_lse):
        xb, wb, b, idx, lse = ctx.saved_tensors
        ext = _require_ext("linear_gather_lse")
        dz = ext.linear_gather_lse_bwd(xb, wb, b, idx, lse, g_val.float().contiguous(),
                                       g_lse.float().contiguous())
        need = ctx.needs_input_grad
        dx = (dz @ wb).to(ctx.in_dtypes[0]) if need[0] else None
        dw = (dz.t() @ xb).to(ctx.in_dtypes[1]) if need[1] else None
        db = dz.sum(0, dtype=torch.float32).to(ctx.in_dtypes[2]) if need[2] else None
        return dx, dw, db, None, None


def linear_gather_lse(x: torch.Tensor, weight: torch.Tensor, bias: torch.Tensor,
                      idx: torch.Tensor) -> Tuple[torch.Tensor, torch.Tensor]:
    if x.is_cuda and x.shape[-1] % 64 == 0:
        ext = _require_ext("linear_gather_lse")
        if ext is not None and hasattr(ext, "linear_gather_lse_fwd"):
            return _LinearGatherLSE.apply(x, weight, bias, idx.contiguous(), ext)
    z = torch.nn.functional.linear(x, weight, bias)
    return z.gather(-1, idx.unsqueeze(-1)).squeeze(-1), torch.logsumexp(z, dim=-1)


def gathered_linear(x: torch.Tensor, weight: torch.Tensor, bias: torch.Tensor,
                    idx: torch.Tensor) -> torch.Tensor:
    out = (x.float() * weight[idx].float()).sum(-1) + bias[idx].float()
    return out.to(x.dtype)


ACT_CODES = {"none": 0, "gelu": 1, "gelu_new": 2, "relu": 3, "silu": 4}
_ACT_FNS = {
    0: lambda y: y,
    1: torch.nn.functional.gelu,
    2: lambda y: torch.nn.functional.gelu(y, approximate="tanh"),
    3: torch.nn.functional.relu,
    4: torch.nn.functional.silu,
}


def skinny_linear(x: torch.Tensor, weight: torch.Tensor, bias: Optional[torch.Tensor] = None,
                  act: int = 0) -> torch.Tensor:
    K = x.shape[-1]
    M = x.numel() // K
    if (x.is_cuda and not torch.is_grad_enabled() and x.dtype == torch.bfloat16
            and weight.dtype == torch.bfloat16 and M <= 256 and K % 32 == 0):
        if os.environ.get("TRLX_AMD_FP8_DECODE") == "1":
            ext = _require_ext("skinny_gemm_fp8")
            if ext is not None and hasattr(ext, "skinny_gemm_fp8"):
                q = getattr(weight, "_fp8_cache", None)
                if q is None or q[0].shape != weight.shape:
                    weight._fp8_cache = quantize_fp8_rows(weight)
                    q = weight._fp8_cache
                bb = bias.bfloat16() if bias is not None and bias.dtype != torch.bfloat16 \
                    else bias
                y = ext.skinny_gemm_fp8(x.reshape(M, K).contiguous(), q[0], q[1], bb, act)
                return y.view(*x.shape[:-1], weight.shape[0])
        if os.environ.get("TRLX_AMD_SKINNY") == "1":
            ext = _require_ext("skinny_gemm")
            if ext is not None and hasattr(ext, "skinny_gemm"):
                y = ext.skinny_gemm(x.reshape(M, K).contiguous(), weight.contiguous(), bias,
                                    act)
                return y.view(*x.shape[:-1], weight.shape[0])
    if (act in (1, 2, 3) and bias is not None and x.is_cuda
            and not torch.is_grad_enabled() and x.dtype == torch.bfloat16
            and _addmm_act_ok()):
        try:
            y = torch._addmm_activation(bias, x.reshape(M, K), weight.t(),
                                        use_gelu=(act != 3))
            return y.view(*x.shape[:-1], weight.shape[0])
        except RuntimeError:
            global _ADDMM_ACT
            _ADDMM_ACT = False
    y = torch.nn.functional.linear(x, weight, bias)
    return _ACT_FNS[act](y)


def quantize_fp8_rows(w: torch.Tensor):
    wf = w.detach().float()
    s = (wf.abs().amax(dim=1) / 448.0).clamp(min=1e-12)
    q = (wf / s[:, None]).clamp(-448.0, 448.0).to(torch.float8_e4m3fn)
    return q.view(torch.uint8).contiguous(), s.contiguous()


def dequantize_fp8_rows(q8: torch.Tensor, s: torch.Tensor) -> torch.Tensor:
    return q8.view(torch.float8_e4m3fn).float() * s[:, None]


def refresh_fp8_caches(module: "torch.nn.Module") -> int:
    n = 0
    for m in module.modules():
        w = getattr(m, "weight", None)
        q = getattr(w, "_fp8_cache", None) if w is not None else None
        if q is not None:
            q8, s = quantize_fp8_rows(w)
            q[0].copy_(q8)
            q[1].copy_(s)
            n += 1
    return n


_ADDMM_ACT: Optional[bool] = None


def _addmm_act_ok() -> bool:
    global _ADDMM_ACT
    if _ADDMM_ACT is None:
        _ADDMM_ACT = (hasattr(torch, "_addmm_activation")
                      and os.environ.get("TRLX_AMD_NO_FUSED_ACT") != "1")
    return _ADDMM_ACT




class _Norm(torch.autograd.Function):

    @staticmethod
    def forward(ctx, kind, x, res, weight, bias, eps, ext):
        x2d = x.reshape(-1, x.shape[-1]).contiguous()
        r2d = res.reshape(x2d.shape).contiguous() if res is not None else None
        if kind == "rmsnorm":
            out, *stats = ext.rmsnorm_fwd(x2d, weight, eps, r2d)
        else:
            out, *stats = ext.layernorm_fwd(x2d, weight, bias, eps, r2d)
        s = stats.pop() if res is not None else x2d
        ctx.save_for_backward(s, weight, *stats)
        ctx.kind = kind
        ctx.x_shape = x.shape
        ctx.has_res = res is not None
        ctx.has_bias = bias is not None
        out = out.view(x.shape)
        return (out, s.view(x.shape)) if res is not None else out

    @staticmethod
    def backward(ctx, grad_out, grad_s=None):
        s2d, weight, *stats = ctx.saved_tensors
        ext = _require_ext(ctx.kind)
        bwd = ext.rmsnorm_bwd if ctx.kind == "rmsnorm" else ext.layernorm_bwd
        gs = grad_s.reshape(s2d.shape).contiguous() if grad_s is not None else None
        dx, dw, *db = bwd(s2d, weight, *stats, grad_out.reshape(s2d.shape).contiguous(), gs)
        dx = dx.view(ctx.x_shape)
        return (None, dx, dx if ctx.has_res else None, dw, db[0] if ctx.has_bias else None,
                None, None)


def rmsnorm(x: torch.Tensor, weight: torch.Tensor, eps: float = 1e-6) -> torch.Tensor:
    if x.is_cuda:
        ext = _require_ext("rmsnorm")
        if ext is not None:
            return _Norm.apply("rmsnorm", x, None, weight, None, eps, ext)
    return reference.rmsnorm(x, weight, eps)


def rmsnorm_add(x: torch.Tensor, res: torch.Tensor, weight: torch.Tensor, eps: float = 1e-6):
    if x.is_cuda:
        ext = _require_ext("rmsnorm")
        if ext is not None:
            return _Norm.apply("rmsnorm", x, res, weight, None, eps, ext)
    s = x + res
    return reference.rmsnorm(s, weight, eps), s


def layernorm(
    x: torch.Tensor, weight: torch.Tensor, bias: Optional[torch.Tensor], eps: float = 1e-5
) -> torch.Tensor:
    if x.is_cuda:
        ext = _require_ext("layernorm")
        if ext is not None:
            return _Norm.apply("layernorm", x, None, weight, bias, eps, ext)
    return reference.layernorm(x, weight, bias, eps)


def layernorm_add(x: torch.Tensor, res: torch.Tensor, weight: torch.Tensor,
                  bias: Optional[torch.Tensor], eps: float = 1e-5):
    if x.is_cuda:
        ext = _require_ext("layernorm")
        if ext is not None:
            return _Norm.apply("layernorm", x, res, weight, bias, eps, ext)
    s = x + res
    return reference.layernorm(s, weight, bias, eps), s




class _Rope(torch.autograd.Function):
    @staticmethod
    def forward(ctx, x, cos, sin, positions, interleaved, rot, ext):
        out = ext.rope_fwd(x.contiguous(), cos, sin, positions, interleaved, False, rot)
        ctx.save_for_backward(cos, sin, positions)
        ctx.interleaved = interleaved
        ctx.rot = rot
        return out

    @staticmethod
    def backward(ctx, grad_out):
        cos, sin, positions = ctx.saved_tensors
        ext = _require_ext("rope")
        dx = ext.rope_fwd(grad_out.contiguous(), cos, sin, positions, ctx.interleaved, True, ctx.rot)
        return dx, None, None, None, None, None, None


def apply_rope(
    q: torch.Tensor,
    k: torch.Tensor,
    cos: torch.Tensor,
    sin: torch.Tensor,
    positions: Optional[torch.Tensor] = None,
    interleaved: bool = False,
    rot: int = 0,
) -> Tuple[torch.Tensor, torch.Tensor]:
    D = q.shape[-1]
    if rot <= 0:
        rot = D
    if positions is None:
        T = q.shape[2]
        positions = torch.arange(T, device=q.device, dtype=torch.int32).expand(q.shape[0], T).contiguous()
    if q.is_cuda:
        ext = _require_ext("rope")
        if ext is not None:
            positions = positions.to(torch.int32).contiguous()
            qo = _Rope.apply(q, cos, sin, positions, interleaved, rot, ext)
            ko = _Rope.apply(k, cos, sin, positions, interleaved, rot, ext)
            return qo, ko
    c = cos[positions.long()]
    s = sin[positions.long()]
    return _rope_ref_positional(q, k, c, s, interleaved, rot)


def _rope_ref_positional(q, k, c, s, interleaved, rot):

    def rotate(x):
        xf = x.float()
        xr = xf[..., :rot]
        if interleaved:
            x1, x2 = xr[..., 0::2], xr[..., 1::2]
        else:
            half = rot // 2
            x1, x2 = xr[..., :half], xr[..., half:]
        cc = c.float().unsqueeze(1)
        ss = s.float().unsqueeze(1)
        o1 = x1 * cc - x2 * ss
        o2 = x2 * cc + x1 * ss
        if interleaved:
            out = torch.stack((o1, o2), dim=-1).flatten(-2)
        else:
            out = torch.cat((o1, o2), dim=-1)
        if rot < x.shape[-1]:
            out = torch.cat((out, xf[..., rot:]), dim=-1)
        return out.to(x.dtype)

    return rotate(q), rotate(k)




def gae_advantages_and_returns(
    values: torch.Tensor,
    rewards: torch.Tensor,
    gamma: float,
    lam: float,
    use_whitening: bool = True,
    distributed: bool = False,
    group=None,
) -> Tuple[torch.Tensor, torch.Tensor]:
    if values.is_cuda:
        ext = _require_ext("gae")
        if ext is not None:
            adv, ret = ext.gae(values.contiguous().float(), rewards.contiguous().float(), gamma, lam)
            if use_whitening:
                adv = whiten(adv, distributed=distributed, group=group)
            return adv.detach(), ret
    with torch.no_grad():
        adv, ret = reference.gae_advantages_and_returns(values, rewards, gamma, lam, use_whitening=False)
        if use_whitening:
            adv = whiten(adv, distributed=distributed, group=group)
        return adv.detach(), ret


def whiten(xs: torch.Tensor, shift_mean: bool = True, distributed: bool = False, group=None) -> torch.Tensor:
    if xs.is_cuda:
        ext = _require_ext("whiten")
        if ext is not None:
            stats = ext.sum_count(xs.contiguous().float())
            if distributed:
                import torch.distributed as dist

                dist.all_reduce(stats, group=group)
            mean = stats[0] / stats[2]
            var = stats[1] / stats[2] - mean * mean
            return ext.normalize(xs.contiguous().float(), mean, var, shift_mean)
    return reference.whiten(xs, shift_mean, distributed, group)



PPO_LOSS_STAT_KEYS = (
    "losses/total_loss", "losses/policy_loss", "losses/value_loss",
    "values/mean", "values/min", "values/max", "values/std", "values/values_error", "values/clipfrac",
    "old_values/mean", "old_values/min", "old_values/max", "old_values/std",
    "returns/mean", "returns/min", "returns/max", "returns/std",
    "policy/approx_kl", "policy/clipfrac", "ratio", "padding_percentage",
)


class _PPOLoss(torch.autograd.Function):

    @staticmethod
    def forward(ctx, logprobs, values, old_logprobs, old_values, advantages, returns, mask,
                cliprange, cliprange_value, vf_coef, ext):
        loss, stats, grads = ext.ppo_loss(logprobs, values, old_logprobs, old_values, advantages,
                                          returns, mask, cliprange, cliprange_value, vf_coef)
        ctx.save_for_backward(grads)
        ctx.mark_non_differentiable(stats)
        return loss, stats

    @staticmethod
    def backward(ctx, grad_loss, _grad_stats):
        (grads,) = ctx.saved_tensors
        g = grads * grad_loss
        return (g[0] if ctx.needs_input_grad[0] else None,
                g[1] if ctx.needs_input_grad[1] else None) + (None,) * 9


def ppo_loss_fusable(logprobs, values, old_logprobs, old_values, advantages, returns, mask) -> bool:
    if os.environ.get("TRLX_AMD_NO_FUSED_PPO_LOSS") == "1":
        return False
    floats = (logprobs, values, old_logprobs, old_values, advantages, returns)
    if not (logprobs.is_cuda and logprobs.dim() == 2 and logprobs.numel() > 0):
        return False
    if not all(t.is_cuda and t.dtype == torch.float32 and t.shape == logprobs.shape
               and t.device == logprobs.device for t in floats):
        return False
    if not (mask.is_cuda and mask.dtype == torch.int64 and mask.shape == logprobs.shape
            and mask.device == logprobs.device):
        return False
    if torch.is_grad_enabled() and any(t.requires_grad for t in floats[2:]):
        return False
    return _require_ext("ppo_loss") is not None


def ppo_loss(logprobs, values, old_logprobs, old_values, advantages, returns, mask,
             cliprange: float, cliprange_value: float, vf_coef: float):
    ext = _require_ext("ppo_loss")
    loss, stats = _PPOLoss.apply(logprobs, values, old_logprobs, old_values, advantages, returns,
                                 mask, float(cliprange), float(cliprange_value), float(vf_coef), ext)
    return loss, dict(zip(PPO_LOSS_STAT_KEYS, stats.unbind(0)))




def decode_prep(
    qkv: torch.Tensor,
    k_cache: torch.Tensor,
    v_cache: torch.Tensor,
    cache_idx: torch.Tensor,
    num_heads: int,
    cos: Optional[torch.Tensor] = None,
    sin: Optional[torch.Tensor] = None,
    key_starts: Optional[torch.Tensor] = None,
    rot: int = 0,
    interleaved: bool = False,
) -> torch.Tensor:
    ext = _require_ext("decode_prep")
    return ext.decode_prep(qkv.contiguous(), k_cache, v_cache, cos, sin, key_starts, cache_idx,
                           num_heads, rot, interleaved)


def fused_decode_attention(
    qkv: torch.Tensor,
    k_cache: torch.Tensor,
    v_cache: torch.Tensor,
    seq_lens: torch.Tensor,
    key_starts: Optional[torch.Tensor],
    cos: Optional[torch.Tensor],
    sin: Optional[torch.Tensor],
    cache_idx: torch.Tensor,
    rot: int,
    interleaved: bool,
    scale: float,
    alibi_slopes: Optional[torch.Tensor] = None,
) -> torch.Tensor:
    ext = _require_ext("fused_decode_attention")
    ks = key_starts.to(torch.int32).contiguous() if key_starts is not None else None
    if cos is not None and cos.dtype != torch.float32:
        cos, sin = cos.float(), sin.float()
    return ext.fused_decode_attention(qkv.contiguous(), k_cache, v_cache,
                                      seq_lens.to(torch.int32).contiguous(), ks, cos, sin,
                                      cache_idx, rot, interleaved, scale, alibi_slopes)


class _QKVPrep(torch.autograd.Function):
    @staticmethod
    def forward(ctx, qkv, num_heads, num_kv_heads, head_dim, cos, sin, pos, qscale, rot,
                interleaved, ext):
        q, k, v = ext.qkv_prep_fwd(qkv, num_heads, num_kv_heads, head_dim, cos, sin, pos,
                                   qscale, rot, interleaved)
        ctx.save_for_backward(*( [cos, sin, pos] if cos is not None else [] ))
        ctx.has_rope = cos is not None
        ctx.qscale = qscale
        ctx.rot = rot
        ctx.interleaved = interleaved
        return q, k, v

    @staticmethod
    def backward(ctx, dq, dk, dv):
        ext = _require_ext("qkv_prep")
        cos = sin = pos = None
        if ctx.has_rope:
            cos, sin, pos = ctx.saved_tensors
        dqkv = ext.qkv_prep_bwd(dq.contiguous(), dk.contiguous(), dv.contiguous(), cos, sin,
                                pos, ctx.qscale, ctx.rot, ctx.interleaved)
        return dqkv, None, None, None, None, None, None, None, None, None, None


def qkv_prep(
    qkv: torch.Tensor,
    num_heads: int,
    num_kv_heads: int,
    head_dim: int,
    cos: Optional[torch.Tensor] = None,
    sin: Optional[torch.Tensor] = None,
    positions: Optional[torch.Tensor] = None,
    qscale: float = 1.0,
    rot: int = 0,
    interleaved: bool = False,
):
    ext = _require_ext("qkv_prep")
    if positions is not None:
        positions = positions.to(torch.int32).contiguous()
    if cos is not None and cos.dtype != torch.float32:
        cos, sin = cos.float(), sin.float()
    return _QKVPrep.apply(qkv.contiguous(), num_heads, num_kv_heads, head_dim, cos, sin,
                          positions, qscale, rot, interleaved, ext)


def sample_token(
    logits: torch.Tensor,
    temperature: float = 1.0,
    top_k: int = 0,
    top_p: float = 1.0,
    generator: Optional[torch.Generator] = None,
    seed: Optional[int] = None,
    offset: int = 0,
) -> torch.Tensor:
    if logits.is_cuda:
        ext = _require_ext("sample_token")
        if ext is not None:
            if temperature == 0.0:
                return torch.argmax(logits, dim=-1)
            if seed is None:
                seed = int(torch.randint(0, 2**31 - 1, (1,), generator=generator).item())
            dev_offset = isinstance(offset, torch.Tensor)
            if top_p is not None and 0.0 < top_p < 1.0:
                def _gumbel(t):
                    if dev_offset:
                        return ext.gumbel_sample_dev(t, 1.0, None, seed, offset)
                    return ext.gumbel_sample(t, 1.0, None, seed, offset)

                lg = logits.float() / max(temperature, 1e-6)
                if top_k and 0 < top_k < logits.shape[-1]:
                    vals, idx = torch.topk(lg, top_k, dim=-1)
                    probs = torch.softmax(vals, dim=-1)
                    cum = probs.cumsum(dim=-1)
                    vals = vals.masked_fill(cum - probs > top_p, float("-inf"))
                    pos = _gumbel(vals.contiguous())
                    return idx.gather(-1, pos.view(-1, 1)).view(pos.shape)
                sorted_logits, _ = torch.sort(lg, descending=True, dim=-1)
                probs = torch.softmax(sorted_logits, dim=-1)
                cum = probs.cumsum(dim=-1)
                keep = (cum - probs <= top_p).sum(-1, keepdim=True).clamp(min=1) - 1
                thr = sorted_logits.gather(-1, keep)
                lg = lg.masked_fill(lg < thr, float("-inf"))
                return _gumbel(lg.contiguous())
            if top_k and 0 < top_k < logits.shape[-1]:
                lg = (logits.float() / max(temperature, 1e-6)).contiguous()
                thr = torch.topk(lg, top_k, dim=-1).values[:, -1].contiguous()
                if dev_offset:
                    return ext.gumbel_sample_dev(lg, 1.0, thr, seed, offset)
                return ext.gumbel_sample(lg, 1.0, thr, seed, offset)
            lg = logits.contiguous() if logits.dtype in (torch.float32, torch.bfloat16) \
                else logits.float().contiguous()
            if dev_offset:
                return ext.gumbel_sample_dev(lg, float(temperature), None, seed, offset)
            return ext.gumbel_sample(lg, float(temperature), None, seed, offset)
    return reference.sample_token(logits, temperature, top_k, top_p, generator)


def _top_p_filter(logits: torch.Tensor, top_p: float) -> torch.Tensor:
    sorted_logits, sorted_idx = torch.sort(logits, descending=True, dim=-1)
    probs = torch.softmax(sorted_logits, dim=-1)
    cum = probs.cumsum(dim=-1)
    remove = cum - probs > top_p
    sorted_logits = sorted_logits.masked_fill(remove, float("-inf"))
    return torch.full_like(logits, float("-inf")).scatter(-1, sorted_idx, sorted_logits)




def attention_decode(
    q: torch.Tensor,
    k_cache: torch.Tensor,
    v_cache: torch.Tensor,
    seq_lens: torch.Tensor,
    scale: float,
    seq_starts: Optional[torch.Tensor] = None,
    alibi_slopes: Optional[torch.Tensor] = None,
) -> torch.Tensor:
    if q.is_cuda:
        ext = _require_ext("attention_decode")
        if ext is not None:
            ss = None if seq_starts is None else seq_starts.to(torch.int32).contiguous()
            return ext.attention_decode(
                q.contiguous(), k_cache.contiguous(), v_cache.contiguous(),
                seq_lens.to(torch.int32).contiguous(), scale, ss, alibi_slopes,
            )
    B, Hq, _, D = q.shape
    Hkv = k_cache.shape[1]
    S = k_cache.shape[2]
    qf = q.float()
    kf = k_cache.float()
    vf = v_cache.float()
    if Hkv != Hq:
        rep = Hq // Hkv
        kf = kf.repeat_interleave(rep, dim=1)
        vf = vf.repeat_interleave(rep, dim=1)
    scores = torch.matmul(qf, kf.transpose(-1, -2)) * scale
    pos = torch.arange(S, device=q.device).view(1, 1, 1, S)
    mask = pos >= seq_lens.view(B, 1, 1, 1)
    if seq_starts is not None:
        mask = mask | (pos < seq_starts.view(B, 1, 1, 1))
    if alibi_slopes is not None:
        key_pos = pos if seq_starts is None else (pos - seq_starts.view(B, 1, 1, 1)).clamp(min=0)
        scores = scores + alibi_slopes.float().view(1, Hq, 1, 1) * key_pos.float()
    scores = scores.masked_fill(mask, float("-inf"))
    probs = torch.softmax(scores, dim=-1)
    return torch.matmul(probs, vf).to(q.dtype)




class _CausalSoftmax(torch.autograd.Function):
    @staticmethod
    def forward(ctx, scores, start_pos, key_starts, ext):
        probs = ext.causal_softmax_fwd(scores.contiguous(), start_pos, key_starts)
        ctx.save_for_backward(probs)
        return probs

    @staticmethod
    def backward(ctx, grad_out):
        (probs,) = ctx.saved_tensors
        ext = _require_ext("causal_softmax")
        return ext.causal_softmax_bwd(probs, grad_out.contiguous()), None, None, None


def causal_softmax(
    scores: torch.Tensor, start_pos: int = 0, key_starts: Optional[torch.Tensor] = None
) -> torch.Tensor:
    if scores.is_cuda:
        ext = _require_ext("causal_softmax")
        if ext is not None:
            if key_starts is not None:
                key_starts = key_starts.to(torch.int32).contiguous()
            return _CausalSoftmax.apply(scores, start_pos, key_starts, ext)
    return reference.causal_softmax(scores, start_pos, key_starts)


def flash_prefill(q, k, v, key_starts=None, start_pos: int = 0, scale: float = 1.0,
                  tk=None, alibi_slopes=None):
    ext = _require_ext("flash_prefill")
    if ext is None or not q.is_cuda:
        return reference.flash_prefill(q, k, v, key_starts, start_pos, scale, tk,
                                       alibi_slopes=alibi_slopes)
    ks = key_starts.to(torch.int32).contiguous() if key_starts is not None else None
    return ext.flash_prefill(q.contiguous(), k, v, ks, int(start_pos), float(scale),
                             int(tk) if tk is not None else 0, alibi_slopes)


class _FlashAttention(torch.autograd.Function):

    @staticmethod
    def forward(ctx, q, k, v, key_starts, alibi_slopes, rel_bias, bias_zero, key_mask, causal,
                start_pos, scale, ext):
        out, lse = ext.flash_prefill_lse(q, k, v, key_starts, start_pos, scale, 0, True,
                                         alibi_slopes, rel_bias, bias_zero, key_mask, causal)
        ctx.save_for_backward(q, k, v, out, lse)
        ctx.bwd_args = (key_starts, scale, alibi_slopes, rel_bias, bias_zero - start_pos,
                        key_mask, causal)
        ctx.ext = ext
        return out

    @staticmethod
    def backward(ctx, dout):
        q, k, v, out, lse = ctx.saved_tensors
        dq, dk, dv = ctx.ext.flash_prefill_bwd(q, k, v, out, dout, lse, *ctx.bwd_args)
        return (dq, dk, dv) + (None,) * 9


def flash_attention(q, k, v, key_starts=None, scale: float = 1.0, alibi_slopes=None):
    ext = _require_ext("flash_attention")
    if ext is None or not q.is_cuda:
        return reference.flash_prefill(q, k, v, key_starts, 0, scale,
                                       alibi_slopes=alibi_slopes).to(q.dtype)
    ks = key_starts.to(torch.int32).contiguous() if key_starts is not None else None
    return _FlashAttention.apply(q.contiguous(), k.contiguous(), v.contiguous(), ks,
                                 alibi_slopes, None, 0, None, True, 0, float(scale), ext)




def t5_rel_bias(table: torch.Tensor, q_len: int, k_len: int, q_offset: int = 0,
                bidirectional: bool = True, num_buckets: int = 32,
                max_distance: int = 128) -> Tuple[torch.Tensor, int]:
    return reference.t5_rel_bias(table, q_len, k_len, q_offset, bidirectional, num_buckets,
                                 max_distance)


def seq2seq_attention(q, k, v, rel_bias=None, bias_zero: int = 0, key_mask=None,
                      causal: bool = False, start_pos: int = 0, scale: float = 1.0):
    if rel_bias is not None and rel_bias.requires_grad and torch.is_grad_enabled():
        raise RuntimeError(
            "seq2seq_attention: rel_bias requires grad, but the kernels produce no bias "
            "gradient; detach it or keep this attention on the eager path")
    ext = _require_ext("seq2seq_attention")
    if ext is None or not q.is_cuda:
        return reference.seq2seq_attention(q, k, v, rel_bias, bias_zero, key_mask, causal,
                                           start_pos, scale).to(q.dtype)
    km = None
    if key_mask is not None:
        km = key_mask if key_mask.dtype == torch.uint8 else (key_mask != 0).to(torch.uint8)
        km = km.contiguous()
    rb = rel_bias.detach() if rel_bias is not None else None
    q, k, v = q.contiguous(), k.contiguous(), v.contiguous()
    needs_grad = torch.is_grad_enabled() and (q.requires_grad or k.requires_grad
                                              or v.requires_grad)
    if not needs_grad:
        return ext.flash_prefill(q, k, v, None, int(start_pos), float(scale), 0, None, rb,
                                 int(bias_zero), km, bool(causal))
    if causal and (start_pos != 0 or q.shape[2] != k.shape[2]):
        raise RuntimeError("seq2seq_attention: causal training needs Tq == Tk and start_pos == 0")
    return _FlashAttention.apply(q, k, v, None, None, rb, int(bias_zero), km, bool(causal),
                                 int(start_pos), float(scale), ext)


def seq2seq_decode_enabled(head_dim: int) -> bool:
    return (head_dim in SEQ2SEQ_DECODE_HEAD_DIMS
            and os.environ.get("TRLX_AMD_NO_S2S_DECODE") != "1")


def seq2seq_decode_attention(q, k_new, v_new, k_cache, v_cache, cache_idx, rel_bias=None,
                             bias_zero: int = 0, scale: float = 1.0):
    B, H, D = k_cache.shape[0], k_cache.shape[1], k_cache.shape[3]
    q, k_new, v_new = (t.reshape(B, H, D) for t in (q, k_new, v_new))
    ext = _require_ext("seq2seq_decode_attention") if q.is_cuda else None
    if ext is None:
        return reference.seq2seq_decode_attention(q, k_new, v_new, k_cache, v_cache, cache_idx,
                                                  rel_bias, bias_zero, scale)
    rb = rel_bias.detach() if rel_bias is not None else None
    return ext.seq2seq_decode_attention(q.contiguous(), k_new.contiguous(), v_new.contiguous(),
                                        k_cache, v_cache, cache_idx, rb, int(bias_zero),
                                        float(scale))


def seq2seq_cross_decode_attention(q, k, v, key_mask=None, scale: float = 1.0):
    ext = _require_ext("seq2seq_cross_decode_attention") if q.is_cuda else None
    if ext is None:
        return reference.seq2seq_cross_decode_attention(q, k, v, key_mask, scale)
    return ext.seq2seq_cross_decode_attention(q.contiguous(), k, v, key_mask, float(scale))
```

Baseline: 980.0.

## Add strided packed-QKV flash attention paths to skip transpose copies

Flash forward and backward kernels now take per-tensor batch, head and row strides instead of assuming contiguous [B,H,T,D]. This lets q/k/v be strided views of a packed QKV projection, with output written in [B,T,H,D] order. The goal is to drop the contiguous() transposes and the output permute around attention. A separate delta kernel and optional preallocated dq/dk/dv outputs let the backward write gradients straight into one packed dqkv buffer. The packed path sits behind PACKED_ATTENTION_DEFAULT=False with an env switch, so the default path only gains stride arguments and extra validation.

```diff
diff --git a/trlx_amd/csrc/attn_host.h b/trlx_amd/csrc/attn_host.h
--- a/trlx_amd/csrc/attn_host.h
+++ b/trlx_amd/csrc/attn_host.h
@@ -2,10 +2,12 @@
 
 #include <ATen/ATen.h>
 
+#include <cstdint>
 #include <string>
 #include <type_traits>
 #include <utility>
 
+#include "common.h"
 #include "dispatch.h"
 
 
@@ -52,6 +54,31 @@
   dispatch_head_dim(kFlashHeadDims, D, op, [&](auto d) {
     dispatch_bool(alibi, [&](auto al) { f(d, al, yes, no, no); });
   });
+}
+
+
+inline AttnStrides attn_strides(const at::Tensor& t, const char* op, const char* what) {
+  TORCH_CHECK(t.is_cuda() && t.dtype() == at::kBFloat16 && t.dim() == 4, op, ": ", what,
+              " must be a bf16 [B,H,T,D] tensor on the GPU");
+  TORCH_CHECK(t.size(3) == 0 || t.stride(3) == 1, op, ": ", what,
+              " needs a contiguous last dimension, got stride ", t.stride(3));
+  int64_t s[3];
+  for (int d = 0; d < 3; ++d) {
+    s[d] = t.size(d) > 1 ? t.stride(d) : 0;
+    TORCH_CHECK((t.size(d) <= 1 || s[d] > 0) && s[d] % 8 == 0, op, ": ", what, " stride ", d,
+                " (", s[d], ") must be a positive multiple of 8 elements");
+  }
+  TORCH_CHECK(reinterpret_cast<uintptr_t>(t.data_ptr()) % 16 == 0, op, ": ", what,
+              " must be 16-byte aligned");
+  const int64_t span = (t.size(1) > 0 ? (t.size(1) - 1) * s[1] : 0) +
+                       (t.size(2) > 0 ? (t.size(2) - 1) * s[2] : 0) + t.size(3);
+  TORCH_CHECK(span <= INT32_MAX && s[0] <= INT32_MAX, op, ": ", what,
+              " spans more than 2^31 elements per batch row");
+  return {(int)s[0], (int)s[1], (int)s[2]};
+}
+
+inline bool same_strides(AttnStrides a, AttnStrides b) {
+  return a.b == b.b && a.h == b.h && a.r == b.r;
 }
 
 
diff --git a/trlx_amd/csrc/bindings.cpp b/trlx_amd/csrc/bindings.cpp
--- a/trlx_amd/csrc/bindings.cpp
+++ b/trlx_amd/csrc/bindings.cpp
@@ -117,7 +117,8 @@
                          double scale, long tk,
                          const c10::optional<at::Tensor>& alibi_slopes,
                          const c10::optional<at::Tensor>& rel_bias, long bias_zero,
-                         const c10::optional<at::Tensor>& key_mask, bool causal);
+                         const c10::optional<at::Tensor>& key_mask, bool causal,
+                         bool out_bthd);
 std::vector<at::Tensor> flash_prefill_lse(const at::Tensor& q, const at::Tensor& k,
                                           const at::Tensor& v,
                                           const c10::optional<at::Tensor>& key_starts,
@@ -125,7 +126,8 @@
                                           bool want_lse,
                                           const c10::optional<at::Tensor>& alibi_slopes,
                                           const c10::optional<at::Tensor>& rel_bias, long bias_zero,
-                                          const c10::optional<at::Tensor>& key_mask, bool causal);
+                                          const c10::optional<at::Tensor>& key_mask, bool causal,
+                                          bool out_bthd);
 std::vector<at::Tensor> flash_prefill_bwd(const at::Tensor& q, const at::Tensor& k,
                                           const at::Tensor& v, const at::Tensor& out,
                                           const at::Tensor& dout, const at::Tensor& lse,
@@ -133,7 +135,12 @@
                                           double scale,
                                           const c10::optional<at::Tensor>& alibi_slopes,
                                           const c10::optional<at::Tensor>& rel_bias, long bias_zero,
-                                          const c10::optional<at::Tensor>& key_mask, bool causal);
+                                          const c10::optional<at::Tensor>& key_mask, bool causal,
+                                          const c10::optional<at::Tensor>& delta,
+                                          const c10::optional<at::Tensor>& dq_out,
+                                          const c10::optional<at::Tensor>& dk_out,
+                                          const c10::optional<at::Tensor>& dv_out);
+at::Tensor flash_bwd_delta(const at::Tensor& dout, const at::Tensor& out);
 at::Tensor seq2seq_decode_attention(const at::Tensor& q, const at::Tensor& k_new,
                                     const at::Tensor& v_new, at::Tensor& k_cache,
                                     at::Tensor& v_cache, const at::Tensor& cache_idx,
@@ -201,17 +208,22 @@
           py::arg("key_starts"), py::arg("start_pos"), py::arg("scale"), py::arg("tk"),
           py::arg("alibi_slopes") = py::none(),
           py::arg("rel_bias") = py::none(), py::arg("bias_zero") = 0,
-          py::arg("key_mask") = py::none(), py::arg("causal") = true);
+          py::arg("key_mask") = py::none(), py::arg("causal") = true,
+          py::arg("out_bthd") = false);
   mod.def("flash_prefill_lse", &flash_prefill_lse, py::arg("q"), py::arg("k"), py::arg("v"),
           py::arg("key_starts"), py::arg("start_pos"), py::arg("scale"), py::arg("tk"),
           py::arg("want_lse"), py::arg("alibi_slopes") = py::none(),
           py::arg("rel_bias") = py::none(), py::arg("bias_zero") = 0,
-          py::arg("key_mask") = py::none(), py::arg("causal") = true);
+          py::arg("key_mask") = py::none(), py::arg("causal") = true,
+          py::arg("out_bthd") = false);
   mod.def("flash_prefill_bwd", &flash_prefill_bwd, py::arg("q"), py::arg("k"), py::arg("v"),
           py::arg("out"), py::arg("dout"), py::arg("lse"), py::arg("key_starts"),
           py::arg("scale"), py::arg("alibi_slopes") = py::none(),
           py::arg("rel_bias") = py::none(), py::arg("bias_zero") = 0,
-          py::arg("key_mask") = py::none(), py::arg("causal") = true);
+          py::arg("key_mask") = py::none(), py::arg("causal") = true,
+          py::arg("delta") = py::none(), py::arg("dq") = py::none(), py::arg("dk") = py::none(),
+          py::arg("dv") = py::none());
+  mod.def("flash_bwd_delta", &flash_bwd_delta, py::arg("dout"), py::arg("out"));
   mod.def("seq2seq_decode_attention", &seq2seq_decode_attention, py::arg("q"), py::arg("k_new"),
           py::arg("v_new"), py::arg("k_cache"), py::arg("v_cache"), py::arg("cache_idx"),
           py::arg("rel_bias") = py::none(), py::arg("bias_zero") = 0, py::arg("scale") = 1.0);
diff --git a/trlx_amd/csrc/common.h b/trlx_amd/csrc/common.h
--- a/trlx_amd/csrc/common.h
+++ b/trlx_amd/csrc/common.h
@@ -190,6 +190,14 @@
 }
 
 
+struct AttnStrides {
+  int b, h, r;
+};
+DEV size_t attn_base(AttnStrides s, int b, int h) {
+  return (size_t)b * (size_t)s.b + (size_t)h * (size_t)s.h;
+}
+
+
 DEV unsigned long long splitmix64(unsigned long long z) {
   z += 0x9e3779b97f4a7c15ull;
   z = (z ^ (z >> 30)) * 0xbf58476d1ce4e5b9ull;
diff --git a/trlx_amd/csrc/flash_backward.hip b/trlx_amd/csrc/flash_backward.hip
--- a/trlx_amd/csrc/flash_backward.hip
+++ b/trlx_amd/csrc/flash_backward.hip
@@ -15,13 +15,13 @@
 typedef __attribute__((ext_vector_type(4))) float f32x4_fb;
 
 template <int D, int ST>
-DEV void stage_tileT(const bf16_t* __restrict__ src, long row0, long nrows,
+DEV void stage_tileT(const bf16_t* __restrict__ src, int rstride, int row0, int nrows,
                      unsigned short* __restrict__ tds, float mul) {
   constexpr int KPAD = ST + 8;
   for (int i = threadIdx.x; i < ST * (D / 8); i += BBLOCK) {
     const int row = i / (D / 8);
     const int col = (i % (D / 8)) * 8;
-    const bf16_t* p = src + (size_t)(row0 + min((long)row, nrows - 1)) * D + col;
+    const bf16_t* p = src + (row0 + min(row, nrows - 1)) * rstride + col;
     bf16x8_fb v8 = *reinterpret_cast<const bf16x8_fb*>(p);
 #pragma unroll
     for (int j = 0; j < 8; ++j) {
@@ -32,13 +32,13 @@
 }
 
 template <int D>
-DEV void load_afrag(const bf16_t* __restrict__ src, long row0, long rowmax, int lane,
+DEV void load_afrag(const bf16_t* __restrict__ src, int rstride, int row0, int rowmax, int lane,
                     bf16x8_fb* frag, float mul) {
-  const long row = min(row0 + (long)(lane & 15), rowmax);
+  const int row = min(row0 + (lane & 15), rowmax);
   const int g8 = (lane >> 4) * 8;
 #pragma unroll
   for (int dch = 0; dch < D / 32; ++dch) {
-    bf16x8_fb v8 = *reinterpret_cast<const bf16x8_fb*>(src + (size_t)row * D + dch * 32 + g8);
+    bf16x8_fb v8 = *reinterpret_cast<const bf16x8_fb*>(src + row * rstride + dch * 32 + g8);
     if (mul != 1.f) {
 #pragma unroll
       for (int j = 0; j < 8; ++j) v8[j] = (short)f2bf(bf2f((unsigned short)v8[j]) * mul);
@@ -63,7 +63,8 @@
     const float* __restrict__ drow, const int* __restrict__ key_starts,
     const float* __restrict__ alibi_slopes ,
     bf16_t* __restrict__ dk, bf16_t* __restrict__ dv, int B, int Hq, int Hkv,
-    int Tq , float scale,
+    int Tq ,
+    AttnStrides sq, AttnStrides skv , AttnStrides sdo, float scale,
     S2S... s2s_args ) {
   static_assert(s2s_pack_ok(!CAUSAL || RELB || KMASK, sizeof...(S2S), 5),
                 "seq2seq arguments: (rel_bias, bias_len, bias_zero, key_mask, Tk) iff a mode is on");
@@ -94,10 +95,8 @@
   __shared__ unsigned short p_lds[BBLOCK / WAVE][16 * KPAD];
 
   bf16x8_fb k_frag[D / 32], v_frag[D / 32];
-  load_afrag<D>(k + ((size_t)b * Hkv + hkv) * (size_t)Tk * D, kt + krow0, (long)Tk - 1, lane,
-                k_frag, 1.f);
-  load_afrag<D>(v + ((size_t)b * Hkv + hkv) * (size_t)Tk * D, kt + krow0, (long)Tk - 1, lane,
-                v_frag, 1.f);
+  load_afrag<D>(k + attn_base(skv, b, hkv), skv.r, kt + krow0, Tk - 1, lane, k_frag, 1.f);
+  load_afrag<D>(v + attn_base(skv, b, hkv), skv.r, kt + krow0, Tk - 1, lane, v_frag, 1.f);
   bool kvis[4] = {true, true, true, true};
   if constexpr (KMASK) {
 #pragma unroll
@@ -116,9 +115,8 @@
     const float slope = ALIBI ? alibi_slopes[hq] : 0.f;
     for (int qt = CAUSAL ? kt : 0; qt < Tq; qt += ST) {
       __syncthreads();
-      stage_tileT<D, ST>(q + ((size_t)b * Hq + hq) * (size_t)Tq * D, qt, Tq - qt, qT_lds, scale);
-      stage_tileT<D, ST>(dout + ((size_t)b * Hq + hq) * (size_t)Tq * D, qt, Tq - qt, doT_lds,
-                         1.f);
+      stage_tileT<D, ST>(q + attn_base(sq, b, hq), sq.r, qt, Tq - qt, qT_lds, scale);
+      stage_tileT<D, ST>(dout + attn_base(sdo, b, hq), sdo.r, qt, Tq - qt, doT_lds, 1.f);
       for (int i = threadIdx.x; i < ST; i += BBLOCK) {
         const int qrow = min(qt + i, Tq - 1);
         l_lds[i] = lse[((size_t)b * Hq + hq) * Tq + qrow];
@@ -196,8 +194,8 @@
     for (int r = 0; r < 4; ++r) {
       const int key = kt + krow0 + (lane >> 4) * 4 + r;
       if (key >= Tk) continue;
-      dv[(((size_t)b * Hkv + hkv) * Tk + key) * D + d * 16 + c].u = f2bf(dv_acc[d][r]);
-      dk[(((size_t)b * Hkv + hkv) * Tk + key) * D + d * 16 + c].u = f2bf(dk_acc[d][r]);
+      dv[attn_base(skv, b, hkv) + key * skv.r + d * 16 + c].u = f2bf(dv_acc[d][r]);
+      dk[attn_base(skv, b, hkv) + key * skv.r + d * 16 + c].u = f2bf(dk_acc[d][r]);
     }
 }
 
@@ -209,7 +207,8 @@
     const float* __restrict__ drow, const int* __restrict__ key_starts,
     const float* __restrict__ alibi_slopes ,
     bf16_t* __restrict__ dq, int B, int Hq, int Hkv,
-    int Tq , float scale,
+    int Tq ,
+    AttnStrides sq , AttnStrides skv, AttnStrides sdo, float scale,
     S2S... s2s_args ) {
   static_assert(s2s_pack_ok(!CAUSAL || RELB || KMASK, sizeof...(S2S), 5),
                 "seq2seq arguments: (rel_bias, bias_len, bias_zero, key_mask, Tk) iff a mode is on");
@@ -239,10 +238,8 @@
   __shared__ unsigned short p_lds[BBLOCK / WAVE][16 * KPAD];
 
   bf16x8_fb q_frag[D / 32], do_frag[D / 32];
-  load_afrag<D>(q + ((size_t)b * Hq + h) * (size_t)Tq * D, qt + qrow0, (long)Tq - 1, lane,
-                q_frag, scale);
-  load_afrag<D>(dout + ((size_t)b * Hq + h) * (size_t)Tq * D, qt + qrow0, (long)Tq - 1, lane,
-                do_frag, 1.f);
+  load_afrag<D>(q + attn_base(sq, b, h), sq.r, qt + qrow0, Tq - 1, lane, q_frag, scale);
+  load_afrag<D>(dout + attn_base(sdo, b, h), sdo.r, qt + qrow0, Tq - 1, lane, do_frag, 1.f);
   float L_r[4], D_r[4];
 #pragma unroll
   for (int r = 0; r < 4; ++r) {
@@ -259,8 +256,8 @@
   const int kt_hi = CAUSAL ? min(Tk, qt + BT) : Tk;
   for (int kt = kt_lo; kt < kt_hi; kt += ST) {
     __syncthreads();
-    stage_tileT<D, ST>(k + ((size_t)b * Hkv + hkv) * (size_t)Tk * D, kt, Tk - kt, kT_lds, 1.f);
-    stage_tileT<D, ST>(v + ((size_t)b * Hkv + hkv) * (size_t)Tk * D, kt, Tk - kt, vT_lds, 1.f);
+    stage_tileT<D, ST>(k + attn_base(skv, b, hkv), skv.r, kt, Tk - kt, kT_lds, 1.f);
+    stage_tileT<D, ST>(v + attn_base(skv, b, hkv), skv.r, kt, Tk - kt, vT_lds, 1.f);
     __syncthreads();
 
     unsigned short* pw = p_lds[wid];
@@ -311,10 +308,66 @@
     for (int r = 0; r < 4; ++r) {
       const int qrow = qt + qrow0 + (lane >> 4) * 4 + r;
       if (qrow >= Tq) continue;
-      dq[(((size_t)b * Hq + h) * Tq + qrow) * D + d * 16 + c].u = f2bf(scale * dq_acc[d][r]);
-    }
-}
-
+      dq[attn_base(sq, b, h) + qrow * sq.r + d * 16 + c].u = f2bf(scale * dq_acc[d][r]);
+    }
+}
+
+constexpr int delta_lanes(int D) { return (D / 8) % 8 == 0 ? 8 : (D / 8) % 4 == 0 ? 4 : 1; }
+
+template <int D>
+__global__ __launch_bounds__(BBLOCK) void flash_bwd_delta_kernel(
+    const bf16_t* __restrict__ dout, const bf16_t* __restrict__ out, float* __restrict__ drow,
+    int Hq, int T, long rows , AttnStrides sdo, AttnStrides so) {
+  constexpr int DL = delta_lanes(D);
+  static_assert(BBLOCK % DL == 0 && WAVE % DL == 0, "a row's lanes stay inside one wave");
+  const long gid = ((long)blockIdx.x * BBLOCK + threadIdx.x) / DL;
+  const int j = threadIdx.x % DL;
+  const long row = min(gid, rows - 1);
+  const int t = (int)(row % T);
+  const int h = (int)((row / T) % Hq);
+  const int b = (int)(row / ((long)T * Hq));
+  const bf16_t* dp = dout + attn_base(sdo, b, h) + t * sdo.r;
+  const bf16_t* op = out + attn_base(so, b, h) + t * so.r;
+  float acc = 0.f;
+#pragma unroll
+  for (int ch = j; ch < D / 8; ch += DL) {
+    float a[8], o[8];
+    load8<bf16_t>(dp + ch * 8, a);
+    load8<bf16_t>(op + ch * 8, o);
+#pragma unroll
+    for (int e = 0; e < 8; ++e) acc += a[e] * o[e];
+  }
+#pragma unroll
+  for (int off = DL / 2; off > 0; off >>= 1) acc += __shfl_xor(acc, off);
+  if (j == 0 && gid < rows) drow[gid] = acc;
+}
+
+at::Tensor launch_delta(const at::Tensor& dout, AttnStrides sdo, const at::Tensor& out,
+                        AttnStrides so) {
+  const int B = out.size(0), Hq = out.size(1), T = out.size(2), D = out.size(3);
+  auto drow = at::empty({B, Hq, T}, out.options().dtype(at::kFloat));
+  const long rows = (long)B * Hq * T;
+  if (rows == 0) return drow;
+  auto stream = c10::hip::getCurrentHIPStream();
+  dispatch_head_dim(kFlashHeadDims, D, "flash_bwd_delta", [&](auto d) {
+    constexpr int DV = decltype(d)::value;
+    const long blocks = (rows * delta_lanes(DV) + BBLOCK - 1) / BBLOCK;
+    flash_bwd_delta_kernel<DV><<<dim3((unsigned)blocks), BBLOCK, 0, stream>>>(
+        reinterpret_cast<const bf16_t*>(dout.data_ptr()),
+        reinterpret_cast<const bf16_t*>(out.data_ptr()), drow.data_ptr<float>(), Hq, T, rows, sdo,
+        so);
+  });
+  HIP_CHECK_LAST();
+  return drow;
+}
+
+}
+
+at::Tensor flash_bwd_delta(const at::Tensor& dout, const at::Tensor& out) {
+  const AttnStrides sdo = attn_strides(dout, "flash_bwd_delta", "dout");
+  const AttnStrides so = attn_strides(out, "flash_bwd_delta", "out");
+  TORCH_CHECK(dout.sizes() == out.sizes(), "flash_bwd_delta: dout and out differ in shape");
+  return launch_delta(dout, sdo, out, so);
 }
 
 std::vector<at::Tensor> flash_prefill_bwd(const at::Tensor& q, const at::Tensor& k,
@@ -326,31 +379,56 @@
                                           const c10::optional<at::Tensor>& rel_bias,
                                           long bias_zero,
                                           const c10::optional<at::Tensor>& key_mask,
-                                          bool causal) {
-  TORCH_CHECK(q.is_cuda() && q.dtype() == at::kBFloat16 && q.dim() == 4 && q.is_contiguous(),
-              "flash_prefill_bwd: q must be contiguous bf16 [B,Hq,T,D]");
-  TORCH_CHECK(k.is_contiguous() && v.is_contiguous() && lse.is_contiguous());
+                                          bool causal, const c10::optional<at::Tensor>& delta,
+                                          const c10::optional<at::Tensor>& dq_out,
+                                          const c10::optional<at::Tensor>& dk_out,
+                                          const c10::optional<at::Tensor>& dv_out) {
+  const char* op = "flash_prefill_bwd";
+  const AttnStrides sq = attn_strides(q, op, "q");
+  const AttnStrides skv = attn_strides(k, op, "k");
+  const AttnStrides so = attn_strides(out, op, "out");
+  const AttnStrides sdo = attn_strides(dout, op, "dout");
+  TORCH_CHECK(v.sizes() == k.sizes() && same_strides(attn_strides(v, op, "v"), skv), op,
+              ": k and v must have the same shape and layout");
   const int B = q.size(0), Hq = q.size(1), T = q.size(2), D = q.size(3);
   const int Hkv = k.size(1), Tk = k.size(2);
   TORCH_CHECK(!causal || Tk == T, "flash_prefill_bwd: training path only (Tk == T)");
-  TORCH_CHECK(Hq % Hkv == 0 && k.size(3) == D && v.sizes() == k.sizes());
-  TORCH_CHECK(out.sizes() == q.sizes() && dout.sizes() == q.sizes() && lse.numel() == (long)B * Hq * T);
-  const float* sl = alibi_slopes_ptr(alibi_slopes, q, Hq, "flash_prefill_bwd");
+  TORCH_CHECK(Hq % Hkv == 0 && k.size(0) == B && k.size(3) == D);
+  TORCH_CHECK(out.sizes() == q.sizes() && dout.sizes() == q.sizes());
+  TORCH_CHECK(lse.is_cuda() && lse.dtype() == at::kFloat && lse.is_contiguous() &&
+                  lse.numel() == (long)B * Hq * T,
+              op, ": lse must be contiguous fp32 [B,Hq,T]");
+  const float* sl = alibi_slopes_ptr(alibi_slopes, q, Hq, op);
   const Seq2SeqArgs s2s =
       seq2seq_args(rel_bias, bias_zero, key_mask, causal, key_starts.has_value(), sl != nullptr,
-                   q, B, Hq, T, Tk, 0, D, "flash_prefill_bwd");
-  const auto ks_t = optional_int_ptr(key_starts, q, B, "flash_prefill_bwd", "key_starts");
+                   q, B, Hq, T, Tk, 0, D, op);
+  const auto ks_t = optional_int_ptr(key_starts, q, B, op, "key_starts");
   const int* ks = ks_t.second;
-  auto dq = at::empty_like(q);
-  auto dk = at::empty_like(k);
-  auto dv = at::empty_like(v);
-  auto dc = dout.contiguous();
-  auto drow = (dc.to(at::kFloat) * out.to(at::kFloat)).sum(-1).contiguous();
+  auto grad_like = [&](const c10::optional<at::Tensor>& given, const at::Tensor& like,
+                       AttnStrides sl_, const char* what) {
+    if (!given.has_value()) return at::empty_strided(like.sizes(), like.strides(), like.options());
+    TORCH_CHECK(given->sizes() == like.sizes() && same_strides(attn_strides(*given, op, what), sl_),
+                op, ": ", what, " must have the shape and layout of its input");
+    return *given;
+  };
+  auto dq = grad_like(dq_out, q, sq, "dq");
+  auto dk = grad_like(dk_out, k, skv, "dk");
+  auto dv = grad_like(dv_out, v, skv, "dv");
+  if (q.numel() == 0 || k.numel() == 0) return {dq, dk, dv};
+  at::Tensor drow;
+  if (delta.has_value()) {
+    TORCH_CHECK(delta->is_cuda() && delta->dtype() == at::kFloat && delta->is_contiguous() &&
+                    delta->numel() == (long)B * Hq * T,
+                op, ": delta must be contiguous fp32 [B,Hq,T]");
+    drow = *delta;
+  } else {
+    drow = launch_delta(dout, sdo, out, so);
+  }
   auto stream = c10::hip::getCurrentHIPStream();
   auto qp = reinterpret_cast<const bf16_t*>(q.data_ptr());
   auto kp = reinterpret_cast<const bf16_t*>(k.data_ptr());
   auto vp = reinterpret_cast<const bf16_t*>(v.data_ptr());
-  auto dop = reinterpret_cast<const bf16_t*>(dc.data_ptr());
+  auto dop = reinterpret_cast<const bf16_t*>(dout.data_ptr());
   auto dqp = reinterpret_cast<bf16_t*>(dq.data_ptr());
   auto dkp = reinterpret_cast<bf16_t*>(dk.data_ptr());
   auto dvp = reinterpret_cast<bf16_t*>(dv.data_ptr());
@@ -360,16 +438,17 @@
   dim3 gq((T + BT - 1) / BT, Hq, B);
   dispatch_flash_mode(
       D, sl != nullptr, s2s.any, causal, s2s.rel_bias != nullptr, s2s.key_mask != nullptr,
-      "flash_prefill_bwd", [&](auto d, auto al, auto ca, auto rb, auto km) {
+      op, [&](auto d, auto al, auto ca, auto rb, auto km) {
         constexpr int DV = decltype(d)::value;
         constexpr bool AL = decltype(al)::value, CA = decltype(ca)::value,
                        RB = decltype(rb)::value, KM = decltype(km)::value;
         auto launch = [&](auto... s2s_pack) {
           flash_bwd_dkv_kernel<DV, AL, CA, RB, KM><<<gk, BBLOCK, 0, stream>>>(
-              qp, kp, vp, dop, lp, drp, ks, sl, dkp, dvp, B, Hq, Hkv, T, (float)scale,
+              qp, kp, vp, dop, lp, drp, ks, sl, dkp, dvp, B, Hq, Hkv, T, sq, skv, sdo,
+              (float)scale, s2s_pack...);
+          flash_bwd_dq_kernel<DV, AL, CA, RB, KM><<<gq, BBLOCK, 0, stream>>>(
+              qp, kp, vp, dop, lp, drp, ks, sl, dqp, B, Hq, Hkv, T, sq, skv, sdo, (float)scale,
               s2s_pack...);
-          flash_bwd_dq_kernel<DV, AL, CA, RB, KM><<<gq, BBLOCK, 0, stream>>>(
-              qp, kp, vp, dop, lp, drp, ks, sl, dqp, B, Hq, Hkv, T, (float)scale, s2s_pack...);
         };
         if constexpr (CA && !RB && !KM) launch();
         else launch(s2s.rel_bias, s2s.bias_len, s2s.bias_zero, s2s.key_mask, Tk);
diff --git a/trlx_amd/csrc/flash_prefill.hip b/trlx_amd/csrc/flash_prefill.hip
--- a/trlx_amd/csrc/flash_prefill.hip
+++ b/trlx_amd/csrc/flash_prefill.hip
@@ -23,8 +23,8 @@
     bf16_t* __restrict__ out,
     float* __restrict__ lse ,
     int B, int Hq, int Hkv, int T, int Tk,
-    int Sk , int start_pos, float scale,
-    S2S... s2s_args) {
+    AttnStrides sq, AttnStrides skv ,
+    AttnStrides so, int start_pos, float scale, S2S... s2s_args) {
   static_assert(s2s_pack_ok(!CAUSAL || RELB || KMASK, sizeof...(S2S), 4),
                 "seq2seq arguments: (rel_bias, bias_len, bias_zero, key_mask) iff a mode is on");
   const S2SView s2s = s2s_view(s2s_args...);
@@ -56,7 +56,7 @@
   bf16x8_fp q_frag[QREG ? D / 32 : 1];
   if constexpr (QREG) {
     const int qrow = min(q0 + wid * 16 + (lane & 15), T - 1);
-    const bf16_t* qp = q + (((size_t)b * Hq + h) * T + qrow) * D + (lane >> 4) * 8;
+    const bf16_t* qp = q + attn_base(sq, b, h) + qrow * sq.r + (lane >> 4) * 8;
 #pragma unroll
     for (int dch = 0; dch < D / 32; ++dch) {
       float vals[8];
@@ -65,13 +65,13 @@
       for (int j = 0; j < 8; ++j) q_frag[dch][j] = (short)f2bf(vals[j] * scale);
     }
   } else {
-    const bf16_t* qp = q + (((size_t)b * Hq + h) * T) * D;
+    const bf16_t* qp = q + attn_base(sq, b, h);
     for (int i = threadIdx.x; i < TQ * (D / 8); i += FBLOCK) {
       const int row = i / (D / 8);
       const int col = (i % (D / 8)) * 8;
       const int qrow = min(q0 + row, T - 1);
       float vals[8];
-      load8<bf16_t>(qp + (size_t)qrow * D + col, vals);
+      load8<bf16_t>(qp + qrow * sq.r + col, vals);
       bf16x8_fp s;
 #pragma unroll
       for (int j = 0; j < 8; ++j) s[j] = (short)f2bf(vals[j] * scale);
@@ -93,8 +93,8 @@
 #pragma unroll
   for (int d = 0; d < D / 16; ++d) oacc[d] = {0.f, 0.f, 0.f, 0.f};
 
-  const bf16_t* kp = k + (((size_t)b * Hkv + hkv) * (size_t)Sk) * D;
-  const bf16_t* vp = v + (((size_t)b * Hkv + hkv) * (size_t)Sk) * D;
+  const bf16_t* kp = k + attn_base(skv, b, hkv);
+  const bf16_t* vp = v + attn_base(skv, b, hkv);
 
   const int kt_lo = (kstart / TK) * TK;
   const int kt_hi = CAUSAL ? min(Tk, qhi_pos + 1) : Tk;
@@ -105,9 +105,9 @@
       const int row = i / (D / 8);
       const int col = (i % (D / 8)) * 8;
       const int krow = min(kt + row, Tk - 1);
-      bf16x8_fp kv8 = *reinterpret_cast<const bf16x8_fp*>(kp + (size_t)krow * D + col);
+      bf16x8_fp kv8 = *reinterpret_cast<const bf16x8_fp*>(kp + krow * skv.r + col);
       *reinterpret_cast<bf16x8_fp*>(&k_lds[row * DPAD + col]) = kv8;
-      bf16x8_fp vv8 = *reinterpret_cast<const bf16x8_fp*>(vp + (size_t)krow * D + col);
+      bf16x8_fp vv8 = *reinterpret_cast<const bf16x8_fp*>(vp + krow * skv.r + col);
 #pragma unroll
       for (int j = 0; j < 8; ++j) vt_lds[(col + j) * KPAD + row] = (unsigned short)vv8[j];
     }
@@ -228,30 +228,11 @@
       if (qrow >= T) continue;
       const float denom = l_row[r] > 0.f ? l_row[r] : 1.f;
       const float val = oacc[d][r] / denom;
-      out[(((size_t)b * Hq + h) * T + qrow) * D + d * 16 + c].u = f2bf(val);
+      out[attn_base(so, b, h) + qrow * so.r + d * 16 + c].u = f2bf(val);
     }
   }
 }
 
-}
-
-std::vector<at::Tensor> flash_prefill_lse(const at::Tensor& q, const at::Tensor& k,
-                                          const at::Tensor& v,
-                                          const c10::optional<at::Tensor>& key_starts,
-                                          long start_pos, double scale, long tk, bool want_lse,
-                                          const c10::optional<at::Tensor>& alibi_slopes,
-                                          const c10::optional<at::Tensor>& rel_bias,
-                                          long bias_zero,
-                                          const c10::optional<at::Tensor>& key_mask, bool causal);
-
-at::Tensor flash_prefill(const at::Tensor& q, const at::Tensor& k, const at::Tensor& v,
-                         const c10::optional<at::Tensor>& key_starts, long start_pos,
-                         double scale, long tk,
-                         const c10::optional<at::Tensor>& alibi_slopes,
-                         const c10::optional<at::Tensor>& rel_bias, long bias_zero,
-                         const c10::optional<at::Tensor>& key_mask, bool causal) {
-  return flash_prefill_lse(q, k, v, key_starts, start_pos, scale, tk, false, alibi_slopes,
-                           rel_bias, bias_zero, key_mask, causal)[0];
 }
 
 std::vector<at::Tensor> flash_prefill_lse(const at::Tensor& q, const at::Tensor& k,
@@ -263,21 +244,25 @@
                                           const c10::optional<at::Tensor>& rel_bias,
                                           long bias_zero,
                                           const c10::optional<at::Tensor>& key_mask,
-                                          bool causal) {
-  TORCH_CHECK(q.is_cuda() && q.dtype() == at::kBFloat16 && q.dim() == 4 && q.is_contiguous());
-  TORCH_CHECK(k.is_contiguous() && v.is_contiguous());
+                                          bool causal, bool out_bthd) {
+  const AttnStrides sq = attn_strides(q, "flash_prefill", "q");
+  const AttnStrides skv = attn_strides(k, "flash_prefill", "k");
+  TORCH_CHECK(v.sizes() == k.sizes() && same_strides(attn_strides(v, "flash_prefill", "v"), skv),
+              "flash_prefill: k and v must have the same shape and layout");
   const int B = q.size(0), Hq = q.size(1), T = q.size(2), D = q.size(3);
   const int Hkv = k.size(1), Sk = k.size(2);
   const int Tk = tk > 0 ? (int)tk : Sk;
   TORCH_CHECK(Tk <= Sk);
-  TORCH_CHECK(k.size(3) == D && Hq % Hkv == 0);
+  TORCH_CHECK(k.size(0) == B && k.size(3) == D && Hq % Hkv == 0);
   const float* sl = alibi_slopes_ptr(alibi_slopes, q, Hq, "flash_prefill");
   const Seq2SeqArgs s2s =
       seq2seq_args(rel_bias, bias_zero, key_mask, causal, key_starts.has_value(), sl != nullptr,
                    q, B, Hq, T, Tk, start_pos, D, "flash_prefill");
-  auto out = at::empty_like(q);
+  auto out = out_bthd ? at::empty({B, T, Hq, D}, q.options()).transpose(1, 2)
+                      : at::empty({B, Hq, T, D}, q.options());
   auto lse = want_lse ? at::empty({B, Hq, T}, q.options().dtype(at::kFloat)) : at::Tensor();
   if (q.numel() == 0) return {out, lse};
+  const AttnStrides so = attn_strides(out, "flash_prefill", "out");
   const auto ks_t = optional_int_ptr(key_starts, q, B, "flash_prefill", "key_starts");
   const int* ks = ks_t.second;
   auto stream = c10::hip::getCurrentHIPStream();
@@ -295,8 +280,8 @@
                        RB = decltype(rb)::value, KM = decltype(km)::value;
         auto launch = [&](auto... s2s_pack) {
           flash_prefill_kernel<DV, AL, CA, RB, KM><<<grid, FBLOCK, 0, stream>>>(
-              qp, kp, vp, ks, sl, op, lp, B, Hq, Hkv, T, Tk, Sk, (int)start_pos, (float)scale,
-              s2s_pack...);
+              qp, kp, vp, ks, sl, op, lp, B, Hq, Hkv, T, Tk, sq, skv, so, (int)start_pos,
+              (float)scale, s2s_pack...);
         };
         if constexpr (CA && !RB && !KM) launch();
         else launch(s2s.rel_bias, s2s.bias_len, s2s.bias_zero, s2s.key_mask);
@@ -304,3 +289,14 @@
   HIP_CHECK_LAST();
   return {out, lse};
 }
+
+at::Tensor flash_prefill(const at::Tensor& q, const at::Tensor& k, const at::Tensor& v,
+                         const c10::optional<at::Tensor>& key_starts, long start_pos,
+                         double scale, long tk,
+                         const c10::optional<at::Tensor>& alibi_slopes,
+                         const c10::optional<at::Tensor>& rel_bias, long bias_zero,
+                         const c10::optional<at::Tensor>& key_mask, bool causal,
+                         bool out_bthd) {
+  return flash_prefill_lse(q, k, v, key_starts, start_pos, scale, tk, false, alibi_slopes,
+                           rel_bias, bias_zero, key_mask, causal, out_bthd)[0];
+}
diff --git a/trlx_amd/models/nn/transformer.py b/trlx_amd/models/nn/transformer.py
--- a/trlx_amd/models/nn/transformer.py
+++ b/trlx_amd/models/nn/transformer.py
@@ -159,6 +159,19 @@
                                            alibi_slopes=ctx.alibi_slopes)
             return project(out)
 
+        flash_common = (
+            T > 1 and x.is_cuda and qkv.dtype == torch.bfloat16
+            and (self.attn_pdrop == 0 or not self.training)
+            and ops.extension_available()
+        )
+        packed = ops.packed_attention_enabled()
+        if (packed and flash_common and self.cfg.position_encoding != "rope"
+                and ctx.prefix_kv is None and kv_cache is None and ctx.start_pos == 0
+                and ops.flash_enabled(self.head_dim, train=torch.is_grad_enabled())):
+            out = ops.flash_attention_qkv(qkv, self.num_heads, self.num_kv_heads, self.head_dim,
+                                          ctx.key_starts, self.scale, ctx.alibi_slopes)
+            return dense(self.o_proj, out)
+
         if x.is_cuda and x.dtype == torch.bfloat16 and ops.extension_available():
             use_rope = self.cfg.position_encoding == "rope"
             cos, sin = rope_tables if use_rope else (None, None)
@@ -189,11 +202,6 @@
             k = k.scatter(2, idx, pk.unsqueeze(0).expand(B_, -1, -1, -1))
             v = v.scatter(2, idx, pv.unsqueeze(0).expand(B_, -1, -1, -1))
 
-        flash_common = (
-            T > 1 and x.is_cuda and q.dtype == torch.bfloat16
-            and (self.attn_pdrop == 0 or not self.training)
-            and ops.extension_available()
-        )
         flash_ok = (
             flash_common and not torch.is_grad_enabled()
             and ops.flash_enabled(self.head_dim, train=False)
@@ -223,7 +231,7 @@
             out = ops.flash_prefill(q.contiguous(), k.contiguous(), v.contiguous(),
                                     ctx.key_starts, ctx.start_pos,
                                     1.0 if pre_scaled else self.scale,
-                                    alibi_slopes=ctx.alibi_slopes)
+                                    alibi_slopes=ctx.alibi_slopes, out_bthd=packed)
             return project(out)
 
         flash_train_ok = (
@@ -233,7 +241,7 @@
         if flash_train_ok:
             out = ops.flash_attention(q, k, v, ctx.key_starts,
                                       1.0 if pre_scaled else self.scale,
-                                      alibi_slopes=ctx.alibi_slopes)
+                                      alibi_slopes=ctx.alibi_slopes, out_bthd=packed)
             return project(out)
 
         if self.num_kv_heads != self.num_heads:
diff --git a/trlx_amd/ops/__init__.py b/trlx_amd/ops/__init__.py
--- a/trlx_amd/ops/__init__.py
+++ b/trlx_amd/ops/__init__.py
@@ -732,24 +732,42 @@
     return reference.causal_softmax(scores, start_pos, key_starts)
 
 
+PACKED_ATTENTION_DEFAULT = False
+
+
+def packed_attention_enabled() -> bool:
+    switch = os.environ.get("TRLX_AMD_NO_PACKED_ATTN")
+    if switch in ("0", "1"):
+        return switch == "0"
+    return PACKED_ATTENTION_DEFAULT
+
+
+def _kernel_layout(t: torch.Tensor) -> torch.Tensor:
+    ok = (t.stride(-1) == 1 and t.data_ptr() % 16 == 0
+          and all(n <= 1 or (s > 0 and s % 8 == 0) for n, s in zip(t.shape[:-1], t.stride()[:-1])))
+    return t if ok else t.contiguous()
+
+
 def flash_prefill(q, k, v, key_starts=None, start_pos: int = 0, scale: float = 1.0,
-                  tk=None, alibi_slopes=None):
+                  tk=None, alibi_slopes=None, out_bthd: bool = False):
     ext = _require_ext("flash_prefill")
     if ext is None or not q.is_cuda:
         return reference.flash_prefill(q, k, v, key_starts, start_pos, scale, tk,
                                        alibi_slopes=alibi_slopes)
     ks = key_starts.to(torch.int32).contiguous() if key_starts is not None else None
-    return ext.flash_prefill(q.contiguous(), k, v, ks, int(start_pos), float(scale),
-                             int(tk) if tk is not None else 0, alibi_slopes)
+    return ext.flash_prefill(_kernel_layout(q), k, v, ks, int(start_pos), float(scale),
+                             int(tk) if tk is not None else 0, alibi_slopes,
+                             out_bthd=bool(out_bthd))
 
 
 class _FlashAttention(torch.autograd.Function):
 
     @staticmethod
     def forward(ctx, q, k, v, key_starts, alibi_slopes, rel_bias, bias_zero, key_mask, causal,
-                start_pos, scale, ext):
+                start_pos, scale, ext, out_bthd=False):
         out, lse = ext.flash_prefill_lse(q, k, v, key_starts, start_pos, scale, 0, True,
-                                         alibi_slopes, rel_bias, bias_zero, key_mask, causal)
+                                         alibi_slopes, rel_bias, bias_zero, key_mask, causal,
+                                         out_bthd)
         ctx.save_for_backward(q, k, v, out, lse)
         ctx.bwd_args = (key_starts, scale, alibi_slopes, rel_bias, bias_zero - start_pos,
                         key_mask, causal)
@@ -759,18 +777,80 @@
     @staticmethod
     def backward(ctx, dout):
         q, k, v, out, lse = ctx.saved_tensors
-        dq, dk, dv = ctx.ext.flash_prefill_bwd(q, k, v, out, dout, lse, *ctx.bwd_args)
-        return (dq, dk, dv) + (None,) * 9
-
-
-def flash_attention(q, k, v, key_starts=None, scale: float = 1.0, alibi_slopes=None):
+        dq, dk, dv = ctx.ext.flash_prefill_bwd(q, k, v, out, _kernel_layout(dout), lse,
+                                               *ctx.bwd_args)
+        return (dq, dk, dv) + (None,) * 10
+
+
+def flash_attention(q, k, v, key_starts=None, scale: float = 1.0, alibi_slopes=None,
+                    out_bthd: bool = False, qkv=None):
     ext = _require_ext("flash_attention")
     if ext is None or not q.is_cuda:
         return reference.flash_prefill(q, k, v, key_starts, 0, scale,
                                        alibi_slopes=alibi_slopes).to(q.dtype)
     ks = key_starts.to(torch.int32).contiguous() if key_starts is not None else None
+    if qkv is not None:
+        return _FlashAttentionQKV.apply(qkv, q.shape[1], k.shape[1], q.shape[3], ks,
+                                        float(scale), alibi_slopes, ext)
     return _FlashAttention.apply(q.contiguous(), k.contiguous(), v.contiguous(), ks,
-                                 alibi_slopes, None, 0, None, True, 0, float(scale), ext)
+                                 alibi_slopes, None, 0, None, True, 0, float(scale), ext,
+                                 bool(out_bthd))
+
+
+def _split_qkv(qkv, num_heads: int, num_kv_heads: int, head_dim: int):
+    B, T, _ = qkv.shape
+    qd, kd = num_heads * head_dim, num_kv_heads * head_dim
+    q = qkv[..., :qd].view(B, T, num_heads, head_dim).transpose(1, 2)
+    k = qkv[..., qd:qd + kd].view(B, T, num_kv_heads, head_dim).transpose(1, 2)
+    v = qkv[..., qd + kd:].view(B, T, num_kv_heads, head_dim).transpose(1, 2)
+    return q, k, v
+
+
+class _FlashAttentionQKV(torch.autograd.Function):
+
+    @staticmethod
+    def forward(ctx, qkv, num_heads, num_kv_heads, head_dim, key_starts, scale, alibi_slopes,
+                ext):
+        q, k, v = _split_qkv(qkv, num_heads, num_kv_heads, head_dim)
+        out, lse = ext.flash_prefill_lse(q, k, v, key_starts, 0, scale, 0, True, alibi_slopes,
+                                         None, 0, None, True, True)
+        ctx.save_for_backward(qkv, out, lse)
+        ctx.heads = (num_heads, num_kv_heads, head_dim)
+        ctx.bwd_args = (key_starts, scale, alibi_slopes)
+        ctx.ext = ext
+        return out
+
+    @staticmethod
+    def backward(ctx, dout):
+        qkv, out, lse = ctx.saved_tensors
+        q, k, v = _split_qkv(qkv, *ctx.heads)
+        dqkv = torch.empty_like(qkv)
+        dq, dk, dv = _split_qkv(dqkv, *ctx.heads)
+        ctx.ext.flash_prefill_bwd(q, k, v, out, _kernel_layout(dout), lse, *ctx.bwd_args, None,
+                                  0, None, True, None, dq, dk, dv)
+        return (dqkv,) + (None,) * 7
+
+
+def flash_attention_qkv(qkv, num_heads: int, num_kv_heads: int, head_dim: int,
+                        key_starts=None, scale: float = 1.0, alibi_slopes=None):
+    B, T, width = qkv.shape
+    if width != (num_heads + 2 * num_kv_heads) * head_dim:
+        raise ValueError(f"flash_attention_qkv: qkv width {width} != (Hq + 2*Hkv) * D = "
+                         f"{(num_heads + 2 * num_kv_heads) * head_dim}")
+    ext = _require_ext("flash_attention_qkv")
+    if ext is None or not qkv.is_cuda:
+        q, k, v = (t.contiguous() for t in _split_qkv(qkv, num_heads, num_kv_heads, head_dim))
+        out = reference.flash_prefill(q, k, v, key_starts, 0, scale, alibi_slopes=alibi_slopes)
+        return out.to(qkv.dtype).transpose(1, 2).reshape(B, T, num_heads * head_dim)
+    qkv = qkv.contiguous()
+    q, k, v = _split_qkv(qkv, num_heads, num_kv_heads, head_dim)
+    if torch.is_grad_enabled():
+        out = flash_attention(q, k, v, key_starts, scale, alibi_slopes=alibi_slopes,
+                              out_bthd=True, qkv=qkv)
+    else:
+        out = flash_prefill(q, k, v, key_starts, 0, scale, alibi_slopes=alibi_slopes,
+                            out_bthd=True)
+    return out.transpose(1, 2).reshape(B, T, num_heads * head_dim)
 
 
 
@@ -806,7 +886,7 @@
     if causal and (start_pos != 0 or q.shape[2] != k.shape[2]):
         raise RuntimeError("seq2seq_attention: causal training needs Tq == Tk and start_pos == 0")
     return _FlashAttention.apply(q, k, v, None, None, rb, int(bias_zero), km, bool(causal),
-                                 int(start_pos), float(scale), ext)
+                                 int(start_pos), float(scale), ext, False)
 
 
 def seq2seq_decode_enabled(head_dim: int) -> bool:
```

New measurement: 952.4. 0.972x the previous value.
